# arangrhie/merfin

Measured on AMD Instinct MI355X. Metric: k-mers evaluated/sec (-hist, k=21), higher is better.
Workload: dtype u64 k-mers / u32 counts / f64 K*

## Files before the change

include/merfin_amd.h:

```cpp
#ifndef MERFIN_AMD_H
#define MERFIN_AMD_H

#include <stddef.h>
#include <stdint.h>

#ifdef __cplusplus
extern "C" {
#endif

#define MFX_OK            0
#define MFX_E_INVAL      -1
#define MFX_E_NOMEM      -2
#define MFX_E_HIP        -3
#define MFX_E_FULL       -4
#define MFX_E_OVERFLOW   -5
#define MFX_E_IO         -6
#define MFX_E_FORMAT     -7
#define MFX_E_NODEVICE   -8
#define MFX_E_NONCANON   -9

const char *mfx_last_error(void);
int         mfx_last_error_code(void);
const char *mfx_version(void);
int         mfx_device_count(void);
// ... 150 lines not shown

typedef struct mfx_reads mfx_reads;
typedef struct mfx_reads_stats {
  uint64_t reads, bases;
  uint64_t kmers;
  uint64_t counted;
  uint64_t dropped;
  uint64_t saturated;
  double   seconds_kernel, seconds_copy;
} mfx_reads_stats;
mfx_reads *mfx_reads_begin(mfx_index *ix, uint64_t batch_bases);
int        mfx_reads_set_filter(mfx_reads *r, uint64_t minV, uint64_t maxV);
int        mfx_reads_add(mfx_reads *r, const char *const *bases, const uint64_t *lens, uint64_t n);
int        mfx_reads_end(mfx_reads *r, mfx_reads_stats *out);

mfx_reads *mfx_reads_begin_all(mfx_index *ix, uint64_t batch_bases);
mfx_reads *mfx_reads_begin_range(mfx_index *ix, uint64_t batch_bases, uint64_t key_lo, uint64_t key_hi);

typedef struct mfx_reads_store mfx_reads_store;
mfx_reads_store *mfx_reads_store_create(int k, uint64_t batch_bases, uint64_t max_bytes);
int  mfx_reads_store_add(mfx_reads_store *s, const char *const *bases, const uint64_t *lens, uint64_t n);
int  mfx_reads_store_info(const mfx_reads_store *s, uint64_t *batches, uint64_t *bytes, uint64_t *reads, uint64_t *n_bases, int *complete);
int  mfx_reads_replay(mfx_reads *r, const mfx_reads_store *s, uint64_t first_batch, uint64_t n_batches);
void mfx_reads_store_free(mfx_reads_store *s);
int        mfx_index_growths(const mfx_index *ix, uint64_t *n, double *seconds, double *rehash_seconds, uint64_t *rehash_bytes);

mfx_seq *mfx_seq_upload(int device, const char *const *bases, const uint64_t *lens, uint32_t ncontigs);
mfx_seq *mfx_seq_from_device(int device, const void *const *d_bases, const uint64_t *lens, uint32_t ncontigs,
                             void *stream);
void     mfx_seq_free(mfx_seq *s);
uint32_t mfx_seq_num_contigs(const mfx_seq *s);
uint64_t mfx_seq_num_bases(const mfx_seq *s);
uint64_t mfx_seq_num_tiles(const mfx_seq *s);
int      mfx_seq_is_packed(const mfx_seq *s);

typedef struct {
  double          peak;
  uint32_t        n_prob;
  const uint32_t *probK;
  const double   *probP;
} mfx_kparams;

typedef struct mfx_eval mfx_eval;

mfx_eval *mfx_eval_create(const mfx_index *ix, const mfx_kparams *kp, uint32_t nbins);
void      mfx_eval_free(mfx_eval *ev);
uint32_t  mfx_eval_nbins(const mfx_eval *ev);
int       mfx_diag_gather_rate(int device, uint64_t table_bytes, double *lines_per_s);
int       mfx_eval_debug_enable(mfx_eval *ev, int on);
int       mfx_eval_debug_counters(mfx_eval *ev, uint64_t *out8);
int       mfx_eval_debug_worklist(mfx_eval *ev, int mode, uint32_t segcap);
int       mfx_eval_debug_worklist_read(mfx_eval *ev, int slot, uint32_t *segs, uint32_t *segcap, uint64_t *counts, uint64_t counts_cap,
                                       void *entries, uint64_t entries_cap, uint64_t *n_entries);

int mfx_debug_traverse_host(const void *clusters, uint64_t ncl, const void *variants, uint64_t nvar, const void *alleles, uint64_t nal,
                            const char *win_text, uint64_t win_bytes, const char *al_text, uint64_t al_bytes, uint64_t text_end,
                            uint64_t path_cap, uint64_t row_cap, uint32_t *np, uint32_t *status, char *text, uint64_t *p_off,
                            uint32_t *p_len, uint32_t *p_nv, uint64_t *p_voff, uint64_t *p_cfirst, int32_t *gt, uint32_t *vidx,
                            uint32_t *vlen);
int mfx_debug_score_paths(mfx_eval *ev, const char *text, uint64_t len, uint64_t npaths, uint64_t nvals, const uint64_t *off,
                          const uint32_t *plen, const uint32_t *nv, const uint64_t *voff, const uint64_t *cfirst, const int32_t *gt,
                          const uint32_t *vidx, const uint32_t *vlen, int need_dk, uint32_t *numM, double *totdk);
int mfx_debug_score_paths_trv(mfx_eval *ev, const char *text, uint64_t len, uint64_t npaths, uint64_t nvals, const uint64_t *off,
                              const uint32_t *plen, const uint32_t *nv, const uint64_t *voff, const uint64_t *cfirst, const int32_t *gt,
                              const uint32_t *vidx, const uint32_t *vlen, const void *clusters, uint64_t ncl, const void *variants,
                              uint64_t nvar, const void *alleles, uint64_t nal, const char *win_text, uint64_t win_bytes,
                              const char *al_text, uint64_t al_bytes, uint64_t text_end, uint64_t path_cap, uint64_t row_cap, int need_dk,
                              uint32_t *numM, double *totdk, uint32_t *np, uint32_t *status, char *text_out, uint64_t *p_off,
                              uint32_t *p_len, uint32_t *p_nv, uint64_t *p_voff, uint64_t *p_cfirst, int32_t *gt_out, uint32_t *vidx_out,
                              uint32_t *vlen_out);

void mfx_getK(const mfx_kparams *kp, uint32_t readV, uint32_t asmV,
              double *readK, double *asmK, double *prob);
double mfx_getKmetric(double readK, double asmK);
double mfx_histoQV(double kval, double ktot, int k);

typedef struct {
  uint64_t  kasm;
  uint64_t  kmissing;
  double    koverCpy;
  uint32_t  undrMax, overMax;
  uint64_t *undr, *over;
  uint32_t  ncontigs;
  uint64_t *contig_kasm;
  uint64_t *contig_kmissing;
} mfx_hist_result;

int  mfx_hist_run(mfx_eval *ev, const mfx_seq *seq, mfx_hist_result *out);
void mfx_hist_result_free(mfx_hist_result *r);

void    *mfx_host_alloc(size_t bytes);
void     mfx_host_free(void *p);
mfx_seq *mfx_seq_create(int device, const uint64_t *lens, uint32_t ncontigs);
int      mfx_hist_run_streamed(mfx_eval *ev, mfx_seq *seq, const char *const *bases, mfx_hist_result *out);
int      mfx_hist_run_streamed_multi(mfx_eval *const *evs, mfx_seq *const *seqs, uint32_t ndev, const char *const *bases, mfx_hist_result *out);
int      mfx_hist_run_streamed_range(mfx_eval *ev, mfx_seq *seq, const char *const *bases, uint64_t tile_begin, uint64_t tile_end,
                                     uint64_t *d_counts, double *d_kover);
int      mfx_hist_stream_share(uint64_t ntiles, uint32_t rank, uint32_t nranks, uint64_t *tile_begin, uint64_t *tile_end);
int      mfx_diag_stream_rates(int device, const char *src, uint64_t n, uint32_t threads, double *enc_gbs, double *link_gbs);
void     mfx_pack_bases(const uint8_t *src, uint64_t n, uint64_t *codes, uint32_t *valid);

mfx_index *mfx_index_replicate(const mfx_index *src, int device);
mfx_seq   *mfx_seq_replicate(const mfx_seq *src, int device);
int        mfx_index_replicate_many(const mfx_index *src, const int *devices, uint32_t n, mfx_index **out);
int        mfx_seq_replicate_many(const mfx_seq *src, const int *devices, uint32_t n, mfx_seq **out);
int        mfx_seq_pack(mfx_seq *seq);
// ... 179 lines not shown
```

merfin_amd/binding.py:

```python
import ctypes as C
import os

import numpy as np

_HERE = os.path.dirname(os.path.abspath(__file__))
TILE = 4096

MFX_ERRORS = {-1: "INVAL", -2: "NOMEM", -3: "HIP", -4: "FULL", -5: "OVERFLOW", -6: "IO", -7: "FORMAT", -8: "NODEVICE", -9: "NONCANON"}
E_NONCANON = -9


class MfxError(RuntimeError):
    def __init__(self, code, msg):
        super().__init__("merfin_amd error %s (%d): %s" % (MFX_ERRORS.get(code, "?"), code, msg))
        self.code = code


def lib_path():
    return os.environ.get("MFX_LIB") or os.path.join(_HERE, "libmerfin_amd.so")


class _KP(C.Structure):
    _fields_ = [("peak", C.c_double), ("n_prob", C.c_uint32),
                ("probK", C.POINTER(C.c_uint32)), ("probP", C.POINTER(C.c_double))]
# ... 3 lines not shown
    _fields_ = [("k", C.c_int), ("canonical", C.c_int), ("capacity", C.c_uint64),
                ("distinct", C.c_uint64), ("bytes", C.c_uint64), ("seq_only", C.c_int), ("compact", C.c_int),
                ("dropped", C.c_uint64)]


class _DbInfo(C.Structure):
    _fields_ = [("k", C.c_int), ("format", C.c_int), ("n_kmers", C.c_uint64), ("placed", C.c_int)]


class _VarOpts(C.Structure):
    _fields_ = [("mode", C.c_int), ("comb", C.c_uint32), ("nosplit", C.c_int), ("debug_path", C.c_char_p)]


INDEX_HEADER_BYTES = 128

VARIANT_MODES = {"filter": 4, "polish": 5, "better": 6, "strict": 7, "loose": 8}


class _ReadsStats(C.Structure):
    _fields_ = [("reads", C.c_uint64), ("bases", C.c_uint64), ("kmers", C.c_uint64), ("counted", C.c_uint64),
                ("dropped", C.c_uint64), ("saturated", C.c_uint64), ("seconds_kernel", C.c_double), ("seconds_copy", C.c_double)]


class _SpectrumPeak(C.Structure):
    _fields_ = [("valley", C.c_uint32), ("main_peak", C.c_uint32), ("haploid_peak", C.c_uint32), ("count_at_peak", C.c_uint64)]


class _HistResult(C.Structure):
    _fields_ = [("kasm", C.c_uint64), ("kmissing", C.c_uint64), ("koverCpy", C.c_double),
                ("undrMax", C.c_uint32), ("overMax", C.c_uint32),
                ("undr", C.POINTER(C.c_uint64)), ("over", C.POINTER(C.c_uint64)),
                ("ncontigs", C.c_uint32),
                ("contig_kasm", C.POINTER(C.c_uint64)), ("contig_kmissing", C.POINTER(C.c_uint64))]


_lib = None

SYMBOLS = [
    "mfx_last_error", "mfx_last_error_code", "mfx_version", "mfx_device_count", "mfx_device_warm", "mfx_device_memory",
    "mfx_index_create", "mfx_index_free", "mfx_index_estimate_gb", "mfx_index_add_read", "mfx_index_add_asm",
    "mfx_index_count_asm", "mfx_index_build_for_hist", "mfx_index_count_claimed", "mfx_hist_run_parts", "mfx_index_create_for_seq", "mfx_index_create_for_seq_lf", "mfx_index_create_lf", "mfx_db_stage_begin", "mfx_index_build_for_hist_staged", "mfx_index_load_db_staged", "mfx_db_stage_free", "mfx_db_stage_boost", "mfx_index_estimate_gb_for_seq", "mfx_index_claim_seq", "mfx_index_value", "mfx_index_get_info", "mfx_index_export",
    "mfx_db_probe", "mfx_index_load_db", "mfx_index_load_db_multi", "mfx_db_write_flat", "mfx_db_convert", "mfx_db_merge", "mfx_db_merge_plan", "mfx_db_join_completeness", "mfx_db_join_spectrum", "mfx_db_join_grain", "mfx_db_join_host", "mfx_db_convert_placed", "mfx_db_write_flat_placed", "mfx_db_place_keys", "mfx_index_save", "mfx_index_load",
    "mfx_index_set_fingerprint", "mfx_index_get_origin",
    "mfx_host_alloc", "mfx_host_free", "mfx_seq_create", "mfx_hist_run_streamed",
    "mfx_hist_run_streamed_multi", "mfx_hist_run_streamed_range", "mfx_hist_stream_share",
    "mfx_index_replicate", "mfx_seq_replicate", "mfx_hist_run_multi", "mfx_hist_run_sharded",
    "mfx_comm_unique_id", "mfx_comm_create", "mfx_comm_free", "mfx_comm_rank", "mfx_comm_size", "mfx_comm_barrier", "mfx_comm_exchange_counts", "mfx_comm_alltoallv",
    "mfx_index_replicate_many", "mfx_seq_replicate_many", "mfx_seq_pack",
    "mfx_hist_allreduce", "mfx_hist_allgather_overflow", "mfx_hist_result_add_overflow",
    "mfx_index_image_header", "mfx_index_create_from_header", "mfx_index_device_image", "mfx_index_commit",
    "mfx_seq_upload", "mfx_seq_from_device", "mfx_seq_free", "mfx_seq_num_contigs", "mfx_seq_num_bases",
    "mfx_seq_num_tiles", "mfx_seq_is_packed",
    "mfx_diag_gather_rate",
    "mfx_eval_create", "mfx_eval_free", "mfx_eval_nbins", "mfx_eval_debug_enable", "mfx_eval_debug_counters", "mfx_eval_debug_worklist", "mfx_eval_debug_worklist_read", "mfx_getK", "mfx_getKmetric", "mfx_histoQV",
    "mfx_hist_run", "mfx_hist_result_free", "mfx_hist_launch", "mfx_hist_launch_cyclic", "mfx_hist_result_from_counts",
    "mfx_hist_take_overflow", "mfx_hist_report", "mfx_diag_stream_rates",
    "mfx_pack_bases", "mfx_host_threads_share", "mfx_dump_values", "mfx_dump_contig", "mfx_dump_values_sharded", "mfx_dump_contig_sharded", "mfx_variants_run_sharded", "mfx_vcf_load", "mfx_vcf_free", "mfx_variants_run_vcf", "mfx_vcf_prepare", "mfx_vcf_path_bound", "mfx_index_claim_paths", "mfx_vcf_prepare_path_index", "mfx_completeness", "mfx_completeness_pieces", "mfx_variants_run",
    "mfx_index_set_shard", "mfx_router_create", "mfx_router_free", "mfx_route_tiles", "mfx_hist_keys_launch",
    "mfx_reads_begin", "mfx_reads_set_filter", "mfx_reads_add", "mfx_reads_end",
    "mfx_reads_begin_all", "mfx_index_growths", "mfx_index_write_db",
    "mfx_reads_begin_range", "mfx_index_key_bins", "mfx_db_writer_open", "mfx_db_writer_append_index", "mfx_db_writer_close", "mfx_db_writer_abort",
    "mfx_db_writer_open_streamed", "mfx_db_writer_append_sorted", "mfx_db_writer_info", "mfx_index_write_db_streamed",
    "mfx_reads_store_create", "mfx_reads_store_add", "mfx_reads_store_info", "mfx_reads_replay", "mfx_reads_store_free",
    "mfx_track_num_windows", "mfx_track_run", "mfx_track_write",
    "mfx_regions_run", "mfx_regions_count", "mfx_regions_tiles_revisited", "mfx_diag_regions_times", "mfx_regions_copy", "mfx_regions_free",
    "mfx_regions_write", "mfx_regions_from_planes_host",
    "mfx_db_merge_except", "mfx_phase_run", "mfx_phase_count", "mfx_phase_copy", "mfx_phase_contig_counts", "mfx_phase_free", "mfx_diag_phase_times", "mfx_phase_write",
    "mfx_phase_from_planes_host",
    "mfx_bin_begin", "mfx_bin_add", "mfx_bin_flush", "mfx_bin_ready", "mfx_bin_take", "mfx_bin_end", "mfx_bin_classify", "mfx_bin_plan_host",
    "mfx_spectrum_run", "mfx_spectrum_peak", "mfx_spectrum_write", "mfx_diag_spectrum_time",
    "mfx_db_trio", "mfx_db_trio_hist", "mfx_db_histogram", "mfx_db_histogram_write", "mfx_db_trio_host",
    "mfx_db_diploid", "mfx_db_diploid_host", "mfx_diploid_write_asm",
    "mfx_debug_traverse_host", "mfx_debug_score_paths", "mfx_debug_score_paths_trv",
]

TRV_CLUSTER_DTYPE = np.dtype([("win_off", "<u8"), ("win_len", "<u4"), ("nv", "<u4"), ("var0", "<u4"), ("path_cap", "<u4"),
                              ("text0", "<u8"), ("path0", "<u8"), ("row0", "<u8"), ("text_cap", "<u4"), ("pad", "<u4")])
TRV_VARIANT_DTYPE = np.dtype([("off", "<u4"), ("reflen", "<u4"), ("na", "<u4"), ("al0", "<u4")])
TRV_ALLELE_DTYPE = np.dtype([("off", "<u8"), ("len", "<u4"), ("pad", "<u4")])
assert (TRV_CLUSTER_DTYPE.itemsize, TRV_VARIANT_DTYPE.itemsize, TRV_ALLELE_DTYPE.itemsize) == (56, 16, 16)
TRV_OK, TRV_RANGE, TRV_ROOM = 0, 1, 2
TRV_MAX_NV, TRV_MAX_PATHS, TRV_MAX_LEN = 8, 64, 640

WORKLIST_DTYPE = np.dtype([("kmer", "<u8"), ("aux", "<u4"), ("w", "<u4")])
assert WORKLIST_DTYPE.itemsize == 16

TRACK_DTYPE = np.dtype([("n_kmers", "<u4"), ("n_missing", "<u4"), ("n_scored", "<u4"), ("n_pos", "<u4"), ("n_neg", "<u4"),
                        ("n_nonfinite", "<u4"), ("sum_readK", "<u8"), ("sum_asmK", "<u8"), ("sum_kstar_lo", "<u8"),
                        ("sum_kstar_hi", "<i8"), ("min_kstar", "<f8"), ("max_kstar", "<f8")])
assert TRACK_DTYPE.itemsize == 72

REGION_DTYPE = np.dtype([("contig", "<u4"), ("cls", "<u4"), ("start", "<u8"), ("end", "<u8"), ("n_kmers", "<u8"), ("sum_readK", "<u8"),
                         ("sum_asmK", "<u8"), ("ext_kstar", "<f8")])
assert REGION_DTYPE.itemsize == 56
REGION_CLASSES = ("missing", "collapsed", "expanded")


class _RegionsOpts(C.Structure):
    _fields_ = [("kstar", C.c_double), ("gap", C.c_uint64), ("min_kmers", C.c_uint64)]


PHASE_DTYPE = np.dtype([("contig", "<u4"), ("hap", "<u4"), ("start", "<u8"), ("end", "<u8"), ("n_hap", "<u8"), ("n_switch", "<u8"),
                        ("n_switch_runs", "<u8")])
assert PHASE_DTYPE.itemsize == 48


class _PhaseOpts(C.Structure):
# ... 81 lines not shown
    L.mfx_db_merge.argtypes = [C.POINTER(C.c_char_p), C.c_uint32, C.c_char_p, C.POINTER(DbMergeOpts), C.POINTER(DbMergeStats)]
    L.mfx_db_merge_except.argtypes = [C.POINTER(C.c_char_p), C.c_uint32, C.POINTER(C.c_char_p), C.c_uint32, C.c_char_p, C.POINTER(DbMergeOpts), C.POINTER(DbMergeStats),
                                      u64p]
    L.mfx_db_merge_plan.argtypes = [C.POINTER(u64p), u64p, C.c_uint32, C.c_int, C.c_uint64, u64p, C.c_uint64, u64p]
    L.mfx_db_join_completeness.argtypes = [C.c_char_p, C.c_char_p, C.POINTER(DbJoinOpts), f64p, f64p, C.POINTER(DbJoinStats)]
    L.mfx_db_join_spectrum.argtypes = [C.c_char_p, C.c_char_p, C.POINTER(DbJoinOpts), u64p, u64p, C.POINTER(DbJoinStats)]
    L.mfx_db_join_grain.argtypes = [C.POINTER(C.c_uint32), C.POINTER(C.c_uint32)]
    L.mfx_db_join_grain.restype = None
    L.mfx_db_join_host.argtypes = [u64p, C.POINTER(C.c_uint32), C.c_uint64, u64p, C.POINTER(C.c_uint32), C.c_uint64, u64p, C.POINTER(C.c_uint32), C.POINTER(C.c_uint32),
                                   C.c_uint64, u64p]
    L.mfx_db_trio.argtypes = [C.c_char_p, C.c_char_p, C.c_char_p, C.c_char_p, C.c_char_p, C.POINTER(DbTrioOpts), u64p, C.POINTER(DbTrioStats)]
    L.mfx_db_trio_hist.argtypes = [C.c_char_p, C.c_char_p, C.c_char_p, C.c_uint32, u64p, C.POINTER(DbTrioStats), C.c_int]
    L.mfx_db_histogram.argtypes = [C.c_char_p, C.c_uint32, u64p, u64p, C.c_int]
    L.mfx_db_histogram_write.argtypes = [u64p, C.c_uint32, C.c_char_p]
    L.mfx_db_trio_host.argtypes = [u64p, C.POINTER(C.c_uint32), C.c_uint64, u64p, C.POINTER(C.c_uint32), C.c_uint64, u64p, C.POINTER(C.c_uint32), C.c_uint64, C.c_int,
                                   C.c_uint32, C.c_uint32, C.c_uint32, C.c_uint32, u64p, C.POINTER(C.c_uint32), u64p, u64p, C.POINTER(C.c_uint32), u64p, u64p,
                                   C.POINTER(DbTrioStats)]
    L.mfx_db_diploid.argtypes = [C.c_char_p, C.c_char_p, C.c_char_p, C.POINTER(DbJoinOpts), u64p, u64p, u64p, C.POINTER(DbDiploidStats), f64p, f64p]
    L.mfx_db_diploid_host.argtypes = [u64p, C.POINTER(C.c_uint32), C.c_uint64, u64p, C.POINTER(C.c_uint32), C.c_uint64, u64p, C.POINTER(C.c_uint32), C.c_uint64, C.c_int,
                                      C.POINTER(DbJoinOpts), u64p, C.POINTER(C.c_uint32), C.POINTER(C.c_uint32), C.POINTER(C.c_uint32), C.c_uint64, u64p, u64p, u64p, u64p,
                                      C.POINTER(DbDiploidStats), f64p, f64p]
    L.mfx_diploid_write_asm.argtypes = [u64p, C.c_uint32, C.c_char_p]
    L.mfx_db_write_flat_placed.argtypes = [C.c_char_p, C.c_int, u64p, u32p, C.c_uint64]
    L.mfx_db_place_keys.argtypes = [C.c_int, vp, C.c_uint64, vp, C.c_int, C.c_int]
    L.mfx_index_load_db_multi.argtypes = [C.POINTER(vp), C.c_uint32, C.c_char_p, C.c_int, C.c_uint64, C.c_uint64]
    L.mfx_index_save.argtypes = [vp, C.c_char_p]
    L.mfx_index_load.restype = vp
    L.mfx_index_load.argtypes = [C.c_char_p, C.c_double, C.c_int]
    L.mfx_index_image_header.argtypes = [vp, vp]
    L.mfx_index_create_from_header.restype = vp
    L.mfx_index_create_from_header.argtypes = [vp, C.c_double, C.c_int]
    L.mfx_index_device_image.argtypes = [vp, C.POINTER(vp), u64p, C.POINTER(vp), u64p]
    L.mfx_index_commit.argtypes = [vp]
    L.mfx_seq_upload.restype = vp
    L.mfx_seq_upload.argtypes = [C.c_int, C.POINTER(C.c_char_p), u64p, C.c_uint32]
    L.mfx_seq_from_device.restype = vp
    L.mfx_seq_from_device.argtypes = [C.c_int, C.POINTER(vp), u64p, C.c_uint32, vp]
    L.mfx_seq_free.argtypes = [vp]
    L.mfx_seq_num_contigs.restype = C.c_uint32
    L.mfx_seq_num_contigs.argtypes = [vp]
    L.mfx_seq_num_bases.restype = C.c_uint64
    L.mfx_seq_num_bases.argtypes = [vp]
    L.mfx_seq_num_tiles.restype = C.c_uint64
    L.mfx_seq_num_tiles.argtypes = [vp]
    L.mfx_eval_create.restype = vp
    L.mfx_eval_create.argtypes = [vp, C.POINTER(_KP), C.c_uint32]
    L.mfx_eval_free.argtypes = [vp]
    L.mfx_eval_nbins.restype = C.c_uint32
    L.mfx_eval_nbins.argtypes = [vp]
    L.mfx_diag_gather_rate.argtypes = [C.c_int, C.c_uint64, C.POINTER(C.c_double)]
    L.mfx_eval_debug_enable.argtypes = [vp, C.c_int]
    L.mfx_eval_debug_counters.argtypes = [vp, u64p]
    L.mfx_eval_debug_worklist.argtypes = [vp, C.c_int, C.c_uint32]
    L.mfx_eval_debug_worklist_read.argtypes = [vp, C.c_int, u32p, u32p, u64p, C.c_uint64, vp, C.c_uint64, u64p]
    L.mfx_getK.argtypes = [C.POINTER(_KP), C.c_uint32, C.c_uint32, f64p, f64p, f64p]
    L.mfx_getKmetric.restype = C.c_double
    L.mfx_getKmetric.argtypes = [C.c_double, C.c_double]
    L.mfx_histoQV.restype = C.c_double
    L.mfx_histoQV.argtypes = [C.c_double, C.c_double, C.c_int]
    L.mfx_hist_run.argtypes = [vp, vp, C.POINTER(_HistResult)]
    L.mfx_hist_result_free.argtypes = [C.POINTER(_HistResult)]
    L.mfx_hist_launch.argtypes = [vp, vp, C.c_uint64, C.c_uint64, vp, vp, vp]
    L.mfx_hist_launch_cyclic.argtypes = [vp, vp, C.c_uint32, C.c_uint32, C.c_uint32, vp, vp, vp]
    L.mfx_hist_result_from_counts.argtypes = [C.c_uint32, u64p, C.c_double, C.c_uint32, C.POINTER(_HistResult)]
    L.mfx_hist_take_overflow.argtypes = [vp, u64p, C.c_uint64, u64p]
    L.mfx_diag_stream_rates.argtypes = [C.c_int, vp, C.c_uint64, C.c_uint32, C.POINTER(C.c_double), C.POINTER(C.c_double)]
    L.mfx_hist_report.argtypes = [C.POINTER(_HistResult), C.c_int, C.c_char_p, C.c_char_p]
    L.mfx_dump_values.argtypes = [vp, vp, C.c_uint32, C.c_uint64, C.c_uint64, u32p, u32p, u64p, u64p]
    L.mfx_dump_contig.argtypes = [vp, vp, C.c_uint32, C.c_char_p, C.c_char_p, C.c_int, u64p, u64p]
    L.mfx_dump_values_sharded.argtypes = [vp, vp, C.c_uint32, C.c_uint32, C.c_uint64, C.c_uint64, u32p, u32p, u64p, u64p]
    L.mfx_dump_contig_sharded.argtypes = [vp, vp, C.c_uint32, C.c_uint32, C.c_char_p, C.c_char_p, C.c_int, u64p, u64p]
    L.mfx_variants_run_sharded.argtypes = [vp, C.c_uint32, C.c_char_p, C.POINTER(C.c_char_p), C.POINTER(C.c_char_p), u64p, C.c_uint32,
                                           C.POINTER(_VarOpts), C.c_char_p, C.c_char_p, u64p]
    L.mfx_completeness.argtypes = [vp, f64p, f64p]
    L.mfx_completeness_pieces.argtypes = [vp, f64p, f64p]
    L.mfx_index_set_shard.argtypes = [vp, C.c_uint32, C.c_uint32]
    L.mfx_router_create.restype = vp
    L.mfx_router_create.argtypes = [vp, C.c_uint32, C.c_uint32]
    L.mfx_router_free.argtypes = [vp]
    L.mfx_route_tiles.argtypes = [vp, vp, C.c_uint64, C.c_uint64, C.c_uint32, vp, vp, vp, u64p, vp]
    L.mfx_hist_keys_launch.argtypes = [vp, vp, vp, C.c_uint64, C.c_uint32, vp, vp, vp]
    L.mfx_variants_run.argtypes = [vp, C.c_char_p, C.POINTER(C.c_char_p), C.POINTER(C.c_char_p), u64p, C.c_uint32,
                                   C.POINTER(_VarOpts), C.c_char_p, C.c_char_p, u64p]
    L.mfx_vcf_load.restype = vp
    L.mfx_vcf_load.argtypes = [C.c_char_p]
    L.mfx_vcf_free.restype = None
    L.mfx_vcf_free.argtypes = [vp]
    L.mfx_variants_run_vcf.argtypes = [vp, vp, C.POINTER(C.c_char_p), C.POINTER(C.c_char_p), u64p, C.c_uint32,
                                       C.POINTER(_VarOpts), C.c_char_p, C.c_char_p, u64p]
    L.mfx_vcf_prepare.argtypes = [vp, C.c_int, C.POINTER(C.c_char_p), C.POINTER(C.c_char_p), u64p, C.c_uint32, C.POINTER(_VarOpts)]
    L.mfx_vcf_path_bound.argtypes = [vp, u64p]
    L.mfx_index_claim_paths.argtypes = [vp, vp, u64p]
    L.mfx_vcf_prepare_path_index.argtypes = [vp, C.c_int, C.POINTER(C.c_char_p), C.POINTER(C.c_char_p), u64p, C.c_uint32, C.POINTER(_VarOpts), C.c_double, C.c_int, C.c_double,
                                             C.POINTER(vp)]
    L.mfx_index_set_fingerprint.argtypes = [vp, C.c_uint64]
    L.mfx_index_get_origin.argtypes = [vp, u64p, u64p, u64p]
    L.mfx_host_threads_share.restype = None
    L.mfx_host_threads_share.argtypes = [C.c_uint]
    L.mfx_pack_bases.restype = None
    L.mfx_pack_bases.argtypes = [vp, C.c_uint64, vp, vp]
    L.mfx_host_alloc.restype = vp
    L.mfx_host_alloc.argtypes = [C.c_size_t]
    L.mfx_host_free.restype = None
    L.mfx_host_free.argtypes = [vp]
    L.mfx_seq_create.restype = vp
    L.mfx_seq_create.argtypes = [C.c_int, u64p, C.c_uint32]
# ... 574 lines not shown
    def commit(self):
        _check(load_library().mfx_index_commit(self.h))

    def replicate(self, device):
        h = _need(load_library().mfx_index_replicate(self.h, device))
        ix = Index(0, 0, device=device, _handle=h)
        ix.k = self.k
        return ix

    def replicate_many(self, devices):
        devs = (C.c_int * len(devices))(*devices)
        out = (C.c_void_p * len(devices))()
        _check(load_library().mfx_index_replicate_many(self.h, devs, len(devices), out))
        res = []
        for d, h in zip(devices, out):
            ix = Index(0, 0, device=d, _handle=h)
            ix.k = self.k
            res.append(ix)
        return res

    def set_fingerprint(self, fp):
        _check(load_library().mfx_index_set_fingerprint(self.h, int(fp)))

    def origin(self):
        a, b, c = C.c_uint64(), C.c_uint64(), C.c_uint64()
        _check(load_library().mfx_index_get_origin(self.h, C.byref(a), C.byref(b), C.byref(c)))
        return a.value, b.value, c.value

    def add_read(self, kmers, values, minV=0, maxV=2**64 - 1):
        if isinstance(kmers, np.ndarray):
            kmers = np.ascontiguousarray(kmers, dtype=np.uint64)
            values = np.ascontiguousarray(values, dtype=np.uint32)
        pk, dev, _k1 = _ptr(kmers)
        pv, _, _k2 = _ptr(values)
        _check(load_library().mfx_index_add_read(self.h, pk, pv, len(kmers), minV, maxV, dev))

    def add_asm(self, kmers, values):
        if isinstance(kmers, np.ndarray):
            kmers = np.ascontiguousarray(kmers, dtype=np.uint64)
            values = np.ascontiguousarray(values, dtype=np.uint32)
        pk, dev, _k1 = _ptr(kmers)
        pv, _, _k2 = _ptr(values)
        _check(load_library().mfx_index_add_asm(self.h, pk, pv, len(kmers), dev))

    def set_shard(self, rank, nranks):
        _check(load_library().mfx_index_set_shard(self.h, rank, nranks))

    def load_db(self, path, side, minV=0, maxV=2**64 - 1):
        _check(load_library().mfx_index_load_db(self.h, path.encode(), side, minV, maxV))

    def count_asm(self, seqs, stream=None):
        _check(load_library().mfx_index_count_asm(self.h, seqs.h, C.c_void_p(stream or 0)))

    def count_reads(self, reads, batch_bases=0, minV=0, maxV=2**64 - 1, chunk=4096):
        return self._count_reads(load_library().mfx_reads_begin, reads, batch_bases, minV, maxV, chunk)

    def count_reads_all(self, reads, batch_bases=0, chunk=4096, minV=0, maxV=2**64 - 1):
        return self._count_reads(load_library().mfx_reads_begin_all, reads, batch_bases, minV, maxV, chunk)

    def count_reads_range(self, reads, key_lo, key_hi, batch_bases=0, chunk=4096):
        L = load_library()
        return self._count_reads(lambda h, bb: L.mfx_reads_begin_range(h, bb, int(key_lo), int(key_hi)), reads, batch_bases, 0, 2**64 - 1, chunk)

    def key_bins(self, side=0):
        bins = np.zeros(4096, dtype=np.uint64)
        n = C.c_uint32(0)
        _check(load_library().mfx_index_key_bins(self.h, int(side), bins.ctypes.data_as(C.POINTER(C.c_uint64)), C.byref(n)))
        return bins[:n.value].copy()

    def growths(self):
        n, b = C.c_uint64(0), C.c_uint64(0)
        s, rs = C.c_double(0), C.c_double(0)
        _check(load_library().mfx_index_growths(self.h, C.byref(n), C.byref(s), C.byref(rs), C.byref(b)))
        return {"growths": n.value, "seconds": s.value, "rehash_seconds": rs.value, "rehash_bytes": b.value}

    def write_db(self, path, side=0, streamed=False):
        n = C.c_uint64(0)
        L = load_library()
        _check((L.mfx_index_write_db_streamed if streamed else L.mfx_index_write_db)(self.h, int(side), str(path).encode(), C.byref(n)))
        return n.value

    def _count_reads(self, begin, reads, batch_bases, minV, maxV, chunk):
        L = load_library()
        recs = [x.encode() if isinstance(x, str) else bytes(x) for x in reads]
        r = _need(begin(self.h, int(batch_bases)))
        rc = L.mfx_reads_set_filter(r, int(minV), int(maxV))
        for o in range(0, len(recs), chunk):
            if rc:
                break
            part = recs[o:o + chunk]
            ptrs = (C.c_char_p * len(part))(*part)
            lens = (C.c_uint64 * len(part))(*[len(x) for x in part])
            try:
                rc = L.mfx_reads_add(r, ptrs, lens, len(part))
            except BaseException:
                L.mfx_reads_end(r, None)
                raise
        msg = L.mfx_last_error().decode() if rc else ""
        st = _ReadsStats()
        rc_end = L.mfx_reads_end(r, C.byref(st))
        if rc:
            raise MfxError(rc, msg)
        _check(rc_end)
        return {f: getattr(st, f) for f, _ in _ReadsStats._fields_}

    def value(self, kmers):
# ... 715 lines not shown
        arr = (C.c_char_p * n)(*contigs)
        lens = np.array([len(c) for c in contigs], dtype=np.uint64)
        o = _VarOpts(VARIANT_MODES[mode], comb, 1 if nosplit else 0, debug_path.encode() if debug_path else None)
        h = C.c_void_p(None)
        _check(load_library().mfx_vcf_prepare_path_index(self.h, int(k), nm, arr, lens.ctypes.data_as(C.POINTER(C.c_uint64)), n, C.byref(o), float(max_gb), int(device),
                                                         float(load_factor), C.byref(h)))
        if not h.value:
            return None
        ix = Index(0, 0, device=device, _handle=h.value)
        ix.k = int(k)
        return ix

    def path_bound(self):
        n = C.c_uint64(0)
        _check(load_library().mfx_vcf_path_bound(self.h, C.byref(n)))
        return n.value

    def claim_paths(self, index):
        n = C.c_uint64(0)
        _check(load_library().mfx_index_claim_paths(index.h, self.h, C.byref(n)))
        return n.value

    def close(self):
        if self.h:
            load_library().mfx_vcf_free(self.h)
            self.h = None

    def __del__(self):
        try:
            self.close()
        except Exception:
            pass


class Evaluator:

    def __init__(self, index, kparams, nbins=0):
        self.index = index
        self.kp = kparams
        self.h = _need(load_library().mfx_eval_create(index.h, C.byref(kparams.c), nbins))

    @property
    def nbins(self):
        return load_library().mfx_eval_nbins(self.h)

    def debug(self, on=True):
        _check(load_library().mfx_eval_debug_enable(self.h, 1 if on else 0))

    def debug_counters(self):
        out = np.zeros(8, dtype=np.uint64)
        _check(load_library().mfx_eval_debug_counters(self.h, out.ctypes.data_as(C.POINTER(C.c_uint64))))
        return {"first_pass": int(out[0]), "second_pass": int(out[1]), "side_table": int(out[2]), "line_scans": int(out[3]),
                "side_not_in_two_slots": int(out[4]), "ended_per_lane": int(out[5]),
                "second_bucket": int(out[6])}

    def debug_worklist(self, mode=1, segcap=0):
        _check(load_library().mfx_eval_debug_worklist(self.h, mode, segcap))

    def debug_worklist_read(self, slot=0):
        L = load_library()
        segs, segcap, n = C.c_uint32(0), C.c_uint32(0), C.c_uint64(0)
        _check(L.mfx_eval_debug_worklist_read(self.h, slot, C.byref(segs), C.byref(segcap), None, 0, None, 0, C.byref(n)))
        counts = np.zeros(segs.value, dtype=np.uint64)
        ent = np.zeros(n.value, dtype=WORKLIST_DTYPE)
        _check(L.mfx_eval_debug_worklist_read(self.h, slot, C.byref(segs), C.byref(segcap), counts.ctypes.data_as(C.POINTER(C.c_uint64)), len(counts),
                                              C.c_void_p(ent.ctypes.data), len(ent), C.byref(n)))
        assert n.value == len(ent) and segs.value == len(counts)
        return segs.value, segcap.value, counts, ent

    def hist(self, seqs):
        r = HistResult()
        _check(load_library().mfx_hist_run(self.h, seqs.h, C.byref(r.c)))
        return r

    def hist_streamed(self, seqs, host_contigs):
        ptrs, keep = _host_ptrs(host_contigs)
        r = HistResult()
        _check(load_library().mfx_hist_run_streamed(self.h, seqs.h, ptrs, C.byref(r.c)))
        return r

    def hist_streamed_range(self, seqs, host_contigs, tile_begin, tile_end, d_counts, d_kover):
        ptrs, keep = _host_ptrs(host_contigs)
        pc = d_counts.data_ptr() if hasattr(d_counts, "data_ptr") else int(d_counts)
        pk = d_kover.data_ptr() if hasattr(d_kover, "data_ptr") else int(d_kover)
        _check(load_library().mfx_hist_run_streamed_range(self.h, seqs.h, ptrs, tile_begin, tile_end, C.c_void_p(pc), C.c_void_p(pk)))

    def hist_launch(self, seqs, tile_begin, tile_end, d_counts, d_kover, stream=None):
        pc = d_counts.data_ptr() if hasattr(d_counts, "data_ptr") else int(d_counts)
        pk = d_kover.data_ptr() if hasattr(d_kover, "data_ptr") else int(d_kover)
        _check(load_library().mfx_hist_launch(self.h, seqs.h, tile_begin, tile_end, C.c_void_p(pc), C.c_void_p(pk),
                                              C.c_void_p(stream or 0)))

    def hist_launch_cyclic(self, seqs, rank, nranks, d_counts, d_kover, block_tiles=256, stream=None):
        p = lambda x: C.c_void_p(x.data_ptr() if hasattr(x, "data_ptr") else int(x))
        _check(load_library().mfx_hist_launch_cyclic(self.h, seqs.h, rank, nranks, block_tiles, p(d_counts), p(d_kover),
                                                     C.c_void_p(stream or 0)))

    def result_from_counts(self, h_counts, kover, ncontigs):
        return result_from_counts(self.nbins, h_counts, kover, ncontigs)

    def take_overflow(self, cap=1 << 20):
        rec = np.zeros(2 * cap, dtype=np.uint64)
        n = C.c_uint64(0)
        _check(load_library().mfx_hist_take_overflow(self.h, rec.ctypes.data_as(C.POINTER(C.c_uint64)), cap, C.byref(n)))
        return rec[:2 * n.value].reshape(-1, 2)

    def hist_keys_launch(self, d_keys, d_contigs, n, ncontigs, d_counts, d_kover, stream=None):
# ... 150 lines not shown
```

merfin_amd/csrc/mfx_api.cpp:

```cpp
#include "mfx_host.h"
#include "mfx_histsum.h"
#include "mfx_place.h"
#include "mfx_kernels.h"
#include "mfx_pipe.h"
#include "mfx_pool.h"
#include "mfx_stream_plan.h"

#include <math.h>
#include <stdarg.h>
#include <stddef.h>
#include <stdio.h>
#include <stdlib.h>
#include <string.h>
#include <unistd.h>

#include <algorithm>
#include <atomic>
#include <chrono>
#include <memory>
#include <mutex>
#include <functional>
#include <condition_variable>
#include <string>
#include <thread>
#include <unordered_map>
#include <vector>

static thread_local char g_err[1024] = "";
static thread_local int  g_err_code = 0;

void mfx_set_error(const char *fmt, ...) {
  va_list ap;
  va_start(ap, fmt);
  vsnprintf(g_err, sizeof(g_err), fmt, ap);
  va_end(ap);
}

int mfx_fail(int code, const char *fmt, ...) {
  va_list ap;
  va_start(ap, fmt);
  vsnprintf(g_err, sizeof(g_err), fmt, ap);
  va_end(ap);
  g_err_code = code;
  return code;
}

extern "C" const char *mfx_last_error(void) { return g_err; }
extern "C" int mfx_last_error_code(void) { return g_err_code; }
extern "C" const char *mfx_version(void) { return "merfin_amd 0.2 (gfx950)"; }

extern "C" int mfx_diag_gather_rate(int device, uint64_t table_bytes, double *lines_per_s) {
  if (!lines_per_s || table_bytes < (1ull << 20)) return mfx_fail(MFX_E_INVAL, "mfx_diag_gather_rate: bad argument");
  if (device < 0 || device >= mfx_device_count()) return mfx_fail(MFX_E_NODEVICE, "HIP device %d not available", device);
  int prev = -1;
  (void)hipGetDevice(&prev);
  MFX_HIP(hipSetDevice(device));
// ... 259 lines not shown
    if (budget > 0) budget = std::max(1.0, budget - (double)ix->side_nlines * MFX_ALIGN);
    ix->nlines = lines_auto(capacity_kmers, budget, slots_line, seq_only);
    if (ix->quot) ix->nlines = std::max(ix->nlines, quot_min_lines(k));
  }
  if (ix->nlines >= (1ull << 32)) {
    mfx_fail(MFX_E_NOMEM, "Not enough memory to load databases.  %lu k-mers need %.0f GB on one GPU; shard the index (mfx_index_set_shard).",
             (unsigned long)capacity_kmers, (double)ix->nlines * MFX_ALIGN / 1e9);
    delete ix;
    return nullptr;
  }
  {
    const char *hm = getenv("MFX_HOME_MODE");
    bool mz = hm ? (strcmp(hm, "plain") != 0) : true;
    const char *ws = getenv("MFX_MZ_W");
    const int w_default = compact ? MFX_MZ_W_COMPACT : MFX_MZ_W_DEFAULT;
    int w = ws ? atoi(ws) : w_default;
    if (w < 1 || w > 5) w = w_default;
    ix->mz_w = (mz && !ix->wide()) ? std::min(w, k) : 0;
    {
      const char *mm = getenv("MFX_MZ_MOD");
      const bool modw = ix->mz_w == 4 || (ix->mz_w == 5 && !ix->quot);
      ix->mz_t = (compact && modw && k >= 13 && !(mm && atoi(mm) == 0)) ? (ix->mz_w == 4 ? ((k + 1) & 3) + 4 : 4 + ((k - 8) % 5)) : 0;
    }
  }
  hipError_t e = hipMalloc((void **)&ix->d_slots, ix->total_lines() * MFX_ALIGN);
  if (e != hipSuccess && ix->nlines > std::max(lines_for(capacity_kmers, slots_line), quot_min_lines(ix->quot ? k : 0))) {
    (void)hipGetLastError();
    ix->nlines = std::max(lines_for(capacity_kmers, slots_line), quot_min_lines(ix->quot ? k : 0));
    e = hipMalloc((void **)&ix->d_slots, ix->total_lines() * MFX_ALIGN);
  }
  if (e != hipSuccess) {
    mfx_fail(MFX_E_NOMEM, "hipMalloc of %.3f GB for the k-mer table failed: %s", need, hipGetErrorString(e));
    delete ix;
    return nullptr;
  }
  if (hipMalloc((void **)&ix->d_meta, MFX_META_WORDS * sizeof(uint64_t)) != hipSuccess ||
      mfx_memset_now(ix->d_meta, 0, MFX_META_WORDS * sizeof(uint64_t)) != hipSuccess ||
      (ix->wide() ? hipMemsetAsync(ix->d_slots, 0, ix->nlines * MFX_ALIGN, nullptr)
       : ix->compact ? hipMemsetAsync(ix->d_slots, 0xff, ix->nlines * MFX_ALIGN, nullptr)
                     : mfx_k_table_init(ix->d_slots, ix->nlines * MFX_SLOTS_LINE, nullptr)) != hipSuccess ||
      (ix->compact && mfx_k_table_init(ix->d_slots + ix->nlines * MFX_SLOTS_LINE, ix->side_nlines * MFX_SLOTS_LINE, nullptr) != hipSuccess) ||
      hipDeviceSynchronize() != hipSuccess) {
    mfx_fail(MFX_E_HIP, "k-mer table initialisation failed: %s", hipGetErrorString(hipGetLastError()));
    mfx_index_free(ix);
    return nullptr;
  }
  return ix;
}

extern "C" void mfx_index_free(mfx_index *ix) {
  if (!ix) return;
  DevGuard g(ix->device);
  mfx_index_ingest_release(ix);
  if (ix->d_slots) (void)hipFree(ix->d_slots);
  if (ix->d_meta) (void)hipFree(ix->d_meta);
  delete ix;
}

static mfx_ingest *ingest_get(mfx_index *ix, uint64_t n);

static int index_check(mfx_index *ix) {
  ix->version++;
  uint64_t meta[5];
  MFX_HIP(hipMemcpy(meta, ix->d_meta, sizeof(meta), hipMemcpyDeviceToHost));
  if (meta[4] != 0)
    return mfx_fail(MFX_E_FORMAT, "the database holds %lu records wider than 2k = %d bits: damaged or not a %d-mer database (none was inserted)",
                    (unsigned long)meta[4], 2 * ix->k, ix->k);
  if (meta[2] != 0)
    return mfx_fail(MFX_E_FULL, "k-mer table full: %lu inserts hit the probe limit (capacity %lu k-mers, %lu stored)",
                    (unsigned long)meta[2], (unsigned long)ix->capacity_kmers, (unsigned long)meta[0]);
  if ((double)meta[0] > 0.92 * (double)(ix->nlines * ix->slots_per_line()))
    return mfx_fail(MFX_E_FULL, "k-mer table over-full: %lu k-mers in %lu slots; create the index with a larger capacity",
                    (unsigned long)meta[0], (unsigned long)(ix->nlines * ix->slots_per_line()));
  if (ix->seq_only && meta[1] != 0)
    return mfx_fail(MFX_E_NONCANON, "the database holds %lu non-canonical k-mers: a sequence-only index keeps one slot per canonical k-mer of the "
                    "sequence and cannot answer value(fmer) + value(rmer) for it; build a full index (mfx_index_create)", (unsigned long)meta[1]);
  return MFX_OK;
}

int mfx_index_check(mfx_index *ix) { return index_check(ix); }

int mfx_reads_claim_error(const mfx_index *ix, const char *who) {
  return mfx_fail(MFX_E_INVAL, "%s: reads were counted into this table of %d-mers (mfx_reads_begin); a table of k > %d claims every k-mer it is "
                  "given, and one claimed now would lack the reads' counts -- give the assembly side before the reads", who, ix->k, MFX_MAX_K_NARROW);
}

constexpr uint64_t MFX_INGEST_CHUNK = 1ull << 24;
constexpr int MFX_INGEST_MAX_LANES = 4, MFX_INGEST_MAX_RING = 64, MFX_INGEST_STREAMS = 4;
struct mfx_ingest {
  struct Lane {
    uint64_t *hk = nullptr;
    uint32_t *hv = nullptr;
    hipEvent_t copied = nullptr;
    bool busy = false;
  } L[MFX_INGEST_MAX_LANES];
  struct Dev {
    uint64_t *dk = nullptr;
    uint32_t *dv = nullptr;
    hipEvent_t done = nullptr;
    bool busy = false;
  } D[MFX_INGEST_MAX_RING];
  hipStream_t cs = nullptr;
  hipStream_t is[MFX_INGEST_STREAMS] = {nullptr, nullptr, nullptr, nullptr};
  hipEvent_t after = nullptr;
  int nl = 2;
  int nd = 2;
// ... 294 lines not shown
    if (!par_pread(fd, (uint8_t *)hk, bytes, off(b0), pool.get())) { mfx_fail(MFX_E_IO, "reading '%s' failed", path); return -1; }
    memcpy(hv, dir + 2 * b0, (nb + 1) * 16);
    const uint64_t base = off(b0), m = std::min<uint64_t>(n - b0 * MFX_DELTA_BLOCK, nb * MFX_DELTA_BLOCK);
    d.kbytes = bytes;
    d.vbytes = (nb + 1) * 16;
    d.launch = [nb, m, base, side, placed](mfx_index *ix, uint64_t *dk, uint32_t *dv, hipStream_t st) {
      return placed ? mfx_k_table_add_placed(ix->view(), dk, reinterpret_cast<const uint64_t *>(dv), (uint32_t)nb, m, base, side, ix->d_meta, st)
                    : mfx_k_table_add_delta(ix->view(), dk, reinterpret_cast<const uint64_t *>(dv), (uint32_t)nb, m, base, side, ix->d_meta, st);
    };
    b0 = b1;
    return 1;
  });
}

static int index_add(mfx_index *ix, const uint64_t *kmers, const uint32_t *values, uint64_t n, int side, int on_device) {
  if (!ix || (n && (!kmers || !values))) return mfx_fail(MFX_E_INVAL, "mfx_index_add: null argument");
  if (ix->reads_counted && ix->wide()) return mfx_reads_claim_error(ix, "mfx_index_add");
  DevGuard g(ix->device);
  const size_t kw = ix->key_words();
  auto table_add = [&](const uint64_t *dk, const uint32_t *dv, uint64_t m, hipStream_t s) {
    return ix->wide() ? mfx_kw_table_add(ix->view(), dk, dv, m, side, ix->d_meta, s) : mfx_k_table_add(ix->view(), dk, dv, m, side, ix->d_meta, s);
  };
  if (on_device) {
    ix->frozen = true;
    MFX_HIP(table_add(kmers, values, n, nullptr));
    MFX_HIP(hipDeviceSynchronize());
    return index_check(ix);
  }
  return index_ingest(ix, n, side, [&](uint64_t o, uint64_t m, uint64_t *hk, uint32_t *hv) {
    par_memcpy((uint8_t *)hk, (const char *)(kmers + o * kw), m * 8 * kw);
    par_memcpy((uint8_t *)hv, (const char *)(values + o), m * 4);
    return true;
  });
}

extern "C" int mfx_index_add_read(mfx_index *ix, const uint64_t *kmers, const uint32_t *values, uint64_t n,
                                  uint64_t minV, uint64_t maxV, int on_device) {
  if (!ix) return mfx_fail(MFX_E_INVAL, "mfx_index_add_read: null index");
  if (ix->reads_counted)
    return mfx_fail(MFX_E_INVAL, "mfx_index_add_read: the read side of this index was counted from reads (mfx_reads_begin); an index takes its "
                    "read counts from one source");
  if (ix->filter_set && (ix->minV != minV || ix->maxV != maxV))
    return mfx_fail(MFX_E_INVAL, "mfx_index_add_read: -min/-max must be the same for every batch of one index");
  ix->minV = minV;
  ix->maxV = maxV;
  ix->filter_set = true;
  return index_add(ix, kmers, values, n, 0, on_device);
}

extern "C" int mfx_index_add_asm(mfx_index *ix, const uint64_t *kmers, const uint32_t *values, uint64_t n, int on_device) {
  return index_add(ix, kmers, values, n, 1, on_device);
}

static int index_count(mfx_index *ix, const mfx_seq *seq, int count, void *stream, const char *who, bool defer = false, bool no_wait = false) {
  if (!ix || !seq) return mfx_fail(MFX_E_INVAL, "%s: null argument", who);
  if (ix->device != seq->device) return mfx_fail(MFX_E_INVAL, "index and sequence live on different devices");
  if (ix->reads_counted && ix->wide()) return mfx_reads_claim_error(ix, who);
  if (ix->seq_only && ix->frozen && count != 2)
    return mfx_fail(MFX_E_INVAL, "%s: this sequence-only index already took counts; its k-mers must all be claimed before the first add / load "
                    "(a k-mer claimed now would have missed them)", who);
  if (count == 2 && (!ix->seq_only || ix->wide())) return mfx_fail(MFX_E_INVAL, "%s: counting claimed k-mers needs a sequence-only index (mfx_index_create_for_seq)", who);
  if (seq->partial) return mfx_seq_partial_error(seq, who);
  const bool from_planes = !ix->wide() && (seq->planes_ok || seq->bases_stale) && !(getenv("MFX_COUNT_ASCII") && atoi(getenv("MFX_COUNT_ASCII")));
  if (!from_planes) if (int erc = mfx_seq_ensure_ascii(seq)) return erc;
  DevGuard g(ix->device);
  mfx_count_args a;
  a.t = ix->view();
  a.bases = seq->d_bases;
  if (from_planes) { a.codes = seq->d_codes; a.valid = seq->d_valid; }
  a.contig_off = seq->d_contig_off;
  a.contig_len = seq->d_contig_len;
  a.tile_start = seq->d_tile_start;
  a.ncontigs = seq->ncontigs;
  a.ntiles = seq->ntiles;
  a.meta = ix->d_meta;
  a.count = count;
  if (ix->seq_only && count != 2) {
    uint32_t d = 0;
    if (int drc = mfx_seq_digest32(seq, &d)) return drc;
    if (ix->seq_digest != 0 && ix->seq_digest != d)
      return mfx_fail(MFX_E_INVAL, "%s: this sequence-only index already claimed the k-mers of another sequence (content digest %08x, this one %08x); "
                      "one such index answers for ONE sequence object -- put the contigs into one mfx_seq", who, ix->seq_digest, d);
    ix->seq_digest = d;
  }
  if (count == 2) ix->frozen = true;
  MFX_HIP(ix->wide() ? mfx_kw_count(a, (hipStream_t)stream) : mfx_k_count(a, (hipStream_t)stream));
  if (no_wait) return MFX_OK;
  if (defer) {
    hipEvent_t ev = nullptr;
    hipError_t e = hipEventCreateWithFlags(&ev, hipEventDisableTiming);
    if (e == hipSuccess) e = hipEventRecord(ev, (hipStream_t)stream);
    mfx_ingest *g = e == hipSuccess ? ingest_get(ix, 1ull << 22) : nullptr;
    if (g) {
      if (g->after) { (void)hipEventSynchronize(g->after); (void)hipEventDestroy(g->after); }
      g->after = ev;
      return MFX_OK;
    }
    if (ev) (void)hipEventDestroy(ev);
    (void)hipGetLastError();
  } else if (ix->seq_only && seq->total_bases >= (256ull << 20)) (void)ingest_get(ix, 1ull << 22);
  MFX_HIP(hipStreamSynchronize((hipStream_t)stream));
  return index_check(ix);
}

static void ingest_settle_after(mfx_index *ix) {
  if (!ix || !ix->ingest || !ix->ingest->after) return;
  DevGuard g(ix->device);
  (void)hipEventSynchronize(ix->ingest->after);
  (void)hipEventDestroy(ix->ingest->after);
  ix->ingest->after = nullptr;
}

extern "C" int mfx_index_count_asm(mfx_index *ix, const mfx_seq *seq, void *stream) {
  return index_count(ix, seq, 1, stream, "mfx_index_count_asm");
}

extern "C" int mfx_index_count_claimed(mfx_index *ix, const mfx_seq *seq, void *stream) {
  return index_count(ix, seq, 2, stream, "mfx_index_count_claimed");
}

extern "C" int mfx_index_build_for_hist(mfx_index *ix, const mfx_seq *seq, const char *read_db_path, uint64_t minV, uint64_t maxV) {
  if (!ix || !seq || !read_db_path) return mfx_fail(MFX_E_INVAL, "mfx_index_build_for_hist: null argument");
  const char *ov = getenv("MFX_BUILD_OVERLAP");
  const bool defer = !(ov && atoi(ov) == 0);
  int rc = index_count(ix, seq, 1, nullptr, "mfx_index_build_for_hist", defer);
  if (rc == MFX_OK) rc = mfx_index_load_db(ix, read_db_path, 0, minV, maxV);
  ingest_settle_after(ix);
  return rc;
}

struct mfx_db_stage {
  int device = 0, fd = -1;
  std::string path;
  mfx_flat_delta_info info;
  std::vector<uint64_t> dir;
  uint64_t off0 = 0, payload_bytes = 0;
  uint8_t *d_payload = nullptr;
  uint64_t *d_dir = nullptr;
// ... 367 lines not shown
      std::fill(tc.begin() + (size_t)s->tile_start[c], tc.begin() + (size_t)s->tile_start[c + 1], c);
    MFX_HIP(hipMalloc((void **)&s->d_tile_contig, (tc.size() ? tc.size() : 1) * sizeof(uint32_t)));
    if (!tc.empty()) MFX_HIP(hipMemcpy(s->d_tile_contig, tc.data(), tc.size() * sizeof(uint32_t), hipMemcpyHostToDevice));
  }
  return MFX_OK;
}


int mfx_seq_partial_error(const mfx_seq *s, const char *who) {
  return mfx_fail(MFX_E_INVAL, "%s: the sequence object holds only the tiles [%lu, %lu) of its %lu (the part one device evaluated in a streamed run over "
                  "several); upload the sequence whole", who, (unsigned long)s->part_lo, (unsigned long)s->part_hi, (unsigned long)s->ntiles);
}

int mfx_seq_ensure_ascii(const mfx_seq *cs) {
  if (cs && cs->partial) return mfx_seq_partial_error(cs, "unpacking the sequence");
  std::lock_guard<std::mutex> lazy(cs->lazy_mu);
  if (!cs->bases_stale && cs->d_bases) return MFX_OK;
  mfx_seq *s = const_cast<mfx_seq *>(cs);
  DevGuard g(s->device);
  if (int rc = seq_need_bases(s)) return rc;
  if (!s->bases_stale) return MFX_OK;
  MFX_HIP(mfx_k_unpack(s->d_codes, s->d_valid, s->d_bases, s->buf_bytes / 32, nullptr));
  MFX_HIP(hipDeviceSynchronize());
  s->bases_stale = false;
  return MFX_OK;
}

void seq_digest_finish(const mfx_seq *s, uint64_t h) {
  for (uint32_t c = 0; c < s->ncontigs; ++c) h = (h ^ s->len[c]) * 0x100000001B3ULL + c;
  const uint32_t f = (uint32_t)(h ^ (h >> 32));
  s->digest = f ? f : 1u;
}

int mfx_seq_digest32(const mfx_seq *s, uint32_t *out) {
  if (s->partial) return mfx_seq_partial_error(s, "the sequence's content digest");
  std::lock_guard<std::mutex> lazy(s->lazy_mu);
  if (s->digest == 0) {
    DevGuard g(s->device);
    uint64_t *d = nullptr, h = 0;
    MFX_HIP(hipMalloc((void **)&d, sizeof(uint64_t)));
    hipError_t e = mfx_memset_now(d, 0, sizeof(uint64_t));
    const bool planes = s->planes_ok || s->bases_stale;
    if (!planes && !s->d_bases) { (void)hipFree(d); if (int rc = seq_need_bases(const_cast<mfx_seq *>(s))) return rc; MFX_HIP(hipMalloc((void **)&d, sizeof(uint64_t))); e = mfx_memset_now(d, 0, sizeof(uint64_t)); }
    if (e == hipSuccess) e = mfx_k_seq_digest(s->d_bases, planes ? s->d_codes : nullptr, planes ? s->d_valid : nullptr, s->buf_bytes / 32, d, nullptr);
    if (e == hipSuccess) e = hipMemcpy(&h, d, sizeof(h), hipMemcpyDeviceToHost);
    (void)hipFree(d);
    if (e != hipSuccess) return mfx_fail(MFX_E_HIP, "sequence digest failed: %s", hipGetErrorString(e));
    seq_digest_finish(s, h);
  }
  *out = s->digest;
  return MFX_OK;
}

thread_local bool t_mfx_path_lookup = false;
int mfx_check_seq_of_index(const mfx_index *ix, const mfx_seq *s, const char *who) {
  if (!ix->seq_only || ix->seq_digest == 0) return MFX_OK;
  if (ix->paths_token) {
    if (t_mfx_path_lookup) return MFX_OK;
    return mfx_fail(MFX_E_INVAL, "%s: this index holds the k-mers of a variant call set's PATHS (mfx_index_claim_paths) and answers the variant modes of that "
                    "call set only; build the index from the sequence (mfx_index_create_for_seq) or use a full index", who);
  }
  uint32_t d = 0;
  if (int rc = mfx_seq_digest32(s, &d)) return rc;
  if (d != ix->seq_digest)
    return mfx_fail(MFX_E_INVAL, "%s: this sequence-only index holds the k-mers of ANOTHER sequence (content digest %08x, this one %08x): "
                    "k-mers it never claimed would read as absent; build the index from this sequence (mfx_index_create_for_seq + "
                    "mfx_index_count_asm / mfx_index_claim_seq) or use a full index", who, ix->seq_digest, d);
  return MFX_OK;
}

static void seq_pack_resident(mfx_seq *s) {
  const char *e = getenv("MFX_SEQ_PACK");
  if ((e && atoi(e) == 0) || !s->d_bases) return;
  const bool timing = getenv("MFX_UPLOAD_TIMING") != nullptr;
  const auto t0 = std::chrono::steady_clock::now();
  const uint64_t pw = seq_plane_words(s);
  const bool ok = mfx_seq_planes_once(
      s, pw,
      [](void **p, size_t bytes) { const bool got = hipMalloc(p, bytes) == hipSuccess; if (!got) { *p = nullptr; (void)hipGetLastError(); } return got; },
      [](void *p) { (void)hipFree(p); },
      [pw](mfx_seq *q) {
        const bool done = mfx_memset_now(q->d_valid, 0, pw * sizeof(uint32_t)) == hipSuccess &&
                          mfx_memset_now(q->d_codes, 0, pw * sizeof(uint64_t)) == hipSuccess &&
                          mfx_k_pack(q->d_bases, q->d_codes, q->d_valid, q->buf_bytes / 32, nullptr) == hipSuccess && hipDeviceSynchronize() == hipSuccess;
        if (!done) (void)hipGetLastError();
        return done;
      });
  if (timing)
    fprintf(stderr, "-- resident sequence: packed planes %s, %.3f s (%.1f MB)\n", ok ? "made" : "NOT made (evaluated from its bytes)",
            std::chrono::duration<double>(std::chrono::steady_clock::now() - t0).count(), pw * 12 / 1e6);
}

extern "C" mfx_seq *mfx_seq_upload(int device, const char *const *bases, const uint64_t *lens, uint32_t ncontigs) {
  if ((ncontigs && (!bases || !lens)) || device < 0 || device >= mfx_device_count()) {
    mfx_fail(device < 0 || device >= mfx_device_count() ? MFX_E_NODEVICE : MFX_E_INVAL,
             "mfx_seq_upload: bad argument (device %d of %d)", device, mfx_device_count());
    return nullptr;
  }
  DevGuard g(device);
  const double t_up0 = std::chrono::duration<double>(std::chrono::steady_clock::now().time_since_epoch()).count();
  mfx_seq *s = seq_layout(device, lens, ncontigs);
  const double t_up1 = std::chrono::duration<double>(std::chrono::steady_clock::now().time_since_epoch()).count();
  bool packed_transport = false;
  {
    const char *asc = getenv("MFX_UPLOAD_ASCII");
    const char *pm = getenv("MFX_UPLOAD_PACKED_MIN");
// ... 297 lines not shown
  if (ntl == 0) return MFX_OK;
  DevGuard g(ev->device);
  int canon = 0;
  int rc = eval_canonical(ev, &canon);
  if (rc) return rc;
  if (!chunk_of_total) {
    if (seq->partial) return mfx_seq_partial_error(seq, "-hist");
    rc = mfx_check_seq_of_index(ev->ix, seq, "-hist");
    if (rc) return rc;
  }
  const char *force = getenv("MFX_FORCE_TWO_STRAND");
  if (force && atoi(force)) canon = 0;
  if (!chunk_of_total) {
    rc = ensure_tile_partials(ev, ntl);
    if (rc) return rc;
  }
  if (seq->bases_stale && ev->ix->wide()) {
    rc = mfx_seq_ensure_ascii(seq);
    if (rc) return rc;
  }
  if (!(seq->planes_ok || seq->bases_stale) && !seq->d_bases) {
    rc = mfx_seq_ensure_ascii(seq);
    if (rc) return rc;
  }
  mfx_hist_args a;
  a.t = ev->ix->view();
  a.canonical = canon;
  a.bases = seq->d_bases;
  if (seq->planes_ok || seq->bases_stale) { a.codes = seq->d_codes; a.valid = seq->d_valid; }
  a.contig_off = seq->d_contig_off;
  a.contig_len = seq->d_contig_len;
  a.tile_start = seq->d_tile_start;
  a.ncontigs = seq->ncontigs;
  a.tile_begin = tile_begin;
  a.tile_end = tile_end;
  a.tile_contig = seq->d_tile_contig;
  a.tile_ctr = ev->d_tile_ctr + ctr_slot;
  a.tile_partials = ev->d_tile_partials + (chunk_of_total ? (tile_begin - partials_tile0) * (MFX_BLOCK / 64) : 0);
  a.n_logical = ntl;
  a.part_rank = part_rank;
  a.part_n = part_n;
  a.part_shift = part_shift;
  a.ks.peak = ev->peak;
  a.ks.n_prob = ev->n_prob;
  a.ks.probK = ev->d_probK;
  a.ks.probP = ev->d_probP;
  a.ks.underq = ev->d_underq;
  a.ks.nbins = ev->nbins;
  a.ks.ncontigs = seq->ncontigs;
  a.ks.counts = d_counts;
  a.ks.partials = ev->d_partials;
  a.ks.ovf = ev->d_ovf;
  a.dbg = ev->d_dbg;
  const char *wl_env = getenv("MFX_HIST_WORKLIST");
  const bool wl_off = (wl_env && atoi(wl_env) == 0) || ev->dbg_wl_mode == 0;
  ev->wl_used_segs[ctr_slot] = ev->wl_used_segcap[ctr_slot] = 0;
  if (a.t.compact && canon && ntl < (1ull << 27) && !wl_off) {
    rc = ensure_worklist(ev, ctr_slot, chunk_of_total ? std::max<uint64_t>(ntl, std::min<uint64_t>(chunk_of_total, (128ull << 20) / MFX_TILE)) : ntl);
    if (rc) return rc;
    const uint64_t segs = std::min<uint64_t>((uint64_t)ev->grid, ntl);
    if (ev->d_wl[ctr_slot] && segs <= MFX_WL_HEADER - 2) {
      a.wl = ev->d_wl[ctr_slot];
      a.wl_segs = (uint32_t)segs;
      a.wl_segcap = (uint32_t)(ev->wl_cap[ctr_slot] / segs);
      if (ev->dbg_wl_mode == 2) a.wl_segcap = std::min(a.wl_segcap, ev->dbg_wl_segcap);
      ev->wl_used_segs[ctr_slot] = a.wl_segs;
      ev->wl_used_segcap[ctr_slot] = a.wl_segcap;
    }
  }
  MFX_HIP(ev->ix->wide() ? mfx_kw_hist(a, (int)std::min<uint64_t>((uint64_t)ev->grid, ntl), (hipStream_t)stream)
                          : mfx_k_hist(a, (int)std::min<uint64_t>((uint64_t)ev->grid, ntl), (hipStream_t)stream));
  if (a.wl) MFX_HIP(mfx_k_hist_rest(a, (int)(a.wl_segs * 4u), (hipStream_t)stream));
  if (chunk_of_total) MFX_HIP(hipMemsetAsync(ev->d_tile_ctr + ctr_slot, 0, sizeof(uint64_t), (hipStream_t)stream));
  else MFX_HIP(mfx_k_sum_tile_partials(ev->d_tile_partials, ntl, d_kover, ev->d_tile_ctr, (hipStream_t)stream, ev->ix->wide() ? 0 : 1));
  return MFX_OK;
}

extern "C" int mfx_hist_launch(mfx_eval *ev, const mfx_seq *seq, uint64_t tile_begin, uint64_t tile_end,
                               uint64_t *d_counts, double *d_kover, void *stream) {
  if (!ev || !seq || !d_counts || !d_kover) return mfx_fail(MFX_E_INVAL, "mfx_hist_launch: null argument");
  if (ev->device != seq->device) return mfx_fail(MFX_E_INVAL, "evaluator and sequence live on different devices");
  if (tile_begin > tile_end || tile_end > seq->ntiles) return mfx_fail(MFX_E_INVAL, "tile range [%lu,%lu) outside [0,%lu)",
                                                                      (unsigned long)tile_begin, (unsigned long)tile_end, (unsigned long)seq->ntiles);
  return hist_launch(ev, seq, tile_begin, tile_end, 0, 1, 0, d_counts, d_kover, stream);
}

extern "C" int mfx_hist_launch_cyclic(mfx_eval *ev, const mfx_seq *seq, uint32_t rank, uint32_t nranks, uint32_t block_tiles,
                                      uint64_t *d_counts, double *d_kover, void *stream) {
  if (!ev || !seq || !d_counts || !d_kover) return mfx_fail(MFX_E_INVAL, "mfx_hist_launch_cyclic: null argument");
  if (ev->device != seq->device) return mfx_fail(MFX_E_INVAL, "evaluator and sequence live on different devices");
  if (nranks == 0 || rank >= nranks || block_tiles == 0 || (block_tiles & (block_tiles - 1)))
    return mfx_fail(MFX_E_INVAL, "mfx_hist_launch_cyclic: rank %u of %u, block of %u tiles (a power of two)", rank, nranks, block_tiles);
  uint32_t shift = 0;
  while ((1u << shift) < block_tiles) ++shift;
  if (nranks == 1) return hist_launch(ev, seq, 0, seq->ntiles, 0, 1, 0, d_counts, d_kover, stream);
  return hist_launch(ev, seq, 0, seq->ntiles, rank, nranks, shift, d_counts, d_kover, stream);
}

hipError_t ovf_reset_hip(mfx_eval *ev, hipStream_t st) {
  const hipError_t e = hipMemsetAsync(ev->d_ovf, 0, (2 + (size_t)MFX_OVF_SLOTS) * sizeof(uint64_t), st);
  return e != hipSuccess ? e : hipMemsetAsync(ev->d_ovf + 2 + MFX_OVF_SLOTS, 0xff, (size_t)MFX_OVF_SLOTS * sizeof(uint64_t), st);
}
int mfx_ovf_reset_async(mfx_eval *ev, hipStream_t st) {
  MFX_HIP(ovf_reset_hip(ev, st));
  return MFX_OK;
}
// ... 1051 lines not shown
```

merfin_amd/csrc/mfx_debug.cpp:

```cpp
#include "mfx_internal.h"
#include "mfx_kernels.h"

#include <stddef.h>
#include <string.h>

static_assert(sizeof(mfx_trv_variant) == 16 && offsetof(mfx_trv_variant, off) == 0 && offsetof(mfx_trv_variant, reflen) == 4 &&
              offsetof(mfx_trv_variant, na) == 8 && offsetof(mfx_trv_variant, al0) == 12, "mfx_trv_variant: layout of the C ABI");
static_assert(sizeof(mfx_trv_allele) == 16 && offsetof(mfx_trv_allele, off) == 0 && offsetof(mfx_trv_allele, len) == 8 &&
              offsetof(mfx_trv_allele, pad) == 12, "mfx_trv_allele: layout of the C ABI");
static_assert(sizeof(mfx_trv_cluster) == 56 && offsetof(mfx_trv_cluster, win_off) == 0 && offsetof(mfx_trv_cluster, win_len) == 8 &&
              offsetof(mfx_trv_cluster, nv) == 12 && offsetof(mfx_trv_cluster, var0) == 16 && offsetof(mfx_trv_cluster, path_cap) == 20 &&
              offsetof(mfx_trv_cluster, text0) == 24 && offsetof(mfx_trv_cluster, path0) == 32 && offsetof(mfx_trv_cluster, row0) == 40 &&
              offsetof(mfx_trv_cluster, text_cap) == 48 && offsetof(mfx_trv_cluster, pad) == 52, "mfx_trv_cluster: layout of the C ABI");

namespace {

int check_tables(const char *who, const mfx_trv_cluster *cl, uint64_t ncl, const mfx_trv_variant *var, uint64_t nvar, const mfx_trv_allele *al, uint64_t nal,
                 uint64_t win_bytes, uint64_t al_bytes, uint64_t text_begin, uint64_t text_end, uint64_t path_cap, uint64_t row_cap, bool every_slot) {
  std::vector<uint8_t> owned(every_slot ? path_cap : 0, 0);
  for (uint64_t c = 0; c < ncl; ++c) {
    const mfx_trv_cluster &C = cl[c];
    if (C.win_off > win_bytes || C.win_len > win_bytes - C.win_off) return mfx_fail(MFX_E_INVAL, "%s: cluster %lu: window outside the window text", who, (unsigned long)c);
    if (C.var0 > nvar || C.nv > nvar - C.var0) return mfx_fail(MFX_E_INVAL, "%s: cluster %lu: variants outside the table", who, (unsigned long)c);
    if (C.text0 < text_begin || C.text0 > text_end || C.text_cap > text_end - C.text0) return mfx_fail(MFX_E_INVAL, "%s: cluster %lu: text room outside [%lu, %lu)", who, (unsigned long)c, (unsigned long)text_begin, (unsigned long)text_end);
// ... 100 lines not shown
  rb.p_off = p_off; rb.p_voff = p_voff; rb.p_cfirst = p_cfirst; rb.p_nv = p_nv;
  rb.vidx = vidx_out; rb.vlen = vlen_out;
  return mfx_score_paths_trv(ev, text, len, &pt, &tb, need_dk, numM, totdk, &rb);
}

extern "C" int mfx_eval_debug_worklist(mfx_eval *ev, int mode, uint32_t segcap) {
  if (!ev) return mfx_fail(MFX_E_INVAL, "mfx_eval_debug_worklist: null argument");
  if (mode < 0 || mode > 2) return mfx_fail(MFX_E_INVAL, "mfx_eval_debug_worklist: mode %d (0 no list, 1 default, 2 segments of at most segcap entries)", mode);
  if (mode == 2 && segcap == 0) return mfx_fail(MFX_E_INVAL, "mfx_eval_debug_worklist: mode 2 with segments of 0 entries (mode 0 turns the list off)");
  ev->dbg_wl_mode = mode;
  ev->dbg_wl_segcap = mode == 2 ? segcap : 0u;
  return MFX_OK;
}

extern "C" int mfx_eval_debug_worklist_read(mfx_eval *ev, int slot, uint32_t *segs, uint32_t *segcap, uint64_t *counts, uint64_t counts_cap, void *entries,
                                            uint64_t entries_cap, uint64_t *n_entries) {
  if (!ev || !segs || !segcap || !n_entries) return mfx_fail(MFX_E_INVAL, "mfx_eval_debug_worklist_read: null argument");
  if (slot < 0 || slot > 1) return mfx_fail(MFX_E_INVAL, "mfx_eval_debug_worklist_read: slot %d (0 or 1)", slot);
  *segs = ev->wl_used_segs[slot];
  *segcap = ev->wl_used_segcap[slot];
  *n_entries = 0;
  if (!*segs) return MFX_OK;
  const uint64_t S = *segs, SC = *segcap;
  if (!ev->d_wl[slot] || S > MFX_WL_HEADER - 2 || S * SC > ev->wl_cap[slot])
    return mfx_fail(MFX_E_INVAL, "mfx_eval_debug_worklist_read: %lu segments of %lu entries do not lie in the list of %lu entries", (unsigned long)S,
                    (unsigned long)SC, (unsigned long)ev->wl_cap[slot]);
  int prev = 0;
  MFX_HIP(hipGetDevice(&prev));
  MFX_HIP(hipSetDevice(ev->device));
  struct Back { int d; ~Back() { (void)hipSetDevice(d); } } back{prev};
  MFX_HIP(hipDeviceSynchronize());
  std::vector<uint64_t> n(S);
  MFX_HIP(hipMemcpy(n.data(), ev->d_wl[slot] + 2, S * sizeof(uint64_t), hipMemcpyDeviceToHost));
  uint64_t total = 0;
  for (uint64_t g = 0; g < S; ++g) {
    if (n[g] > SC) return mfx_fail(MFX_E_INVAL, "mfx_eval_debug_worklist_read: segment %lu counts %lu entries, beyond its %lu", (unsigned long)g, (unsigned long)n[g], (unsigned long)SC);
    total += n[g];
  }
  *n_entries = total;
  if (counts) {
    if (counts_cap < S) return mfx_fail(MFX_E_INVAL, "mfx_eval_debug_worklist_read: %lu segments, the caller's counts hold %lu", (unsigned long)S, (unsigned long)counts_cap);
    memcpy(counts, n.data(), S * sizeof(uint64_t));
  }
  if (entries) {
    if (entries_cap < total) return mfx_fail(MFX_E_INVAL, "mfx_eval_debug_worklist_read: %lu entries, the caller's buffer holds %lu", (unsigned long)total, (unsigned long)entries_cap);
    uint8_t *dst = static_cast<uint8_t *>(entries);
    for (uint64_t g = 0; g < S; ++g) {
      if (n[g]) MFX_HIP(hipMemcpy(dst, ev->d_wl[slot] + MFX_WL_HEADER + 2 * g * SC, n[g] * 16, hipMemcpyDeviceToHost));
      dst += n[g] * 16;
    }
  }
  return MFX_OK;
}
```

merfin_amd/csrc/mfx_internal.h:

```cpp
#pragma once
#include "mfx_traverse.h"

#include <hip/hip_runtime.h>
#include <stdint.h>
#include <mutex>
#include <string>
#include <vector>

#include "../../include/merfin_amd.h"
#include "mfx_kstar.h"
#include "mfx_delta.h"

void mfx_set_error(const char *fmt, ...);
int  mfx_fail(int code, const char *fmt, ...);
#define MFX_HIP(call)                                                                         \
  do {                                                                                        \
    hipError_t e_ = (call);                                                                   \
    if (e_ != hipSuccess)                                                                     \
      return mfx_fail(MFX_E_HIP, "%s failed: %s (%s:%d)", #call, hipGetErrorString(e_), __FILE__, __LINE__); \
  } while (0)
#define MFX_HIP_NULL(call)                                                                    \
  do {                                                                                        \
    hipError_t e_ = (call);                                                                   \
    if (e_ != hipSuccess) {                                                                   \
// ... 62 lines not shown
};
constexpr uint32_t MFX_WSLOTS_LINE = 4;
constexpr int      MFX_MAX_K_NARROW = 31, MFX_MAX_K = 64;

constexpr uint32_t MFX_CSLOTS_LINE = 16;
constexpr uint32_t MFX_CSAT = 2047u;
constexpr int      MFX_MAX_K_COMPACT = 31;
constexpr int      MFX_MAX_K_DIRECT = 21;
constexpr int      MFX_MZ_W_COMPACT = 4;

struct mfx_table_view {
  mfx_slot *slots;
  uint64_t  nlines;
  uint32_t  minV, maxV;
  int       k;
  int       mz_w;
  int       mz_t;
  uint32_t  shard_rank, shard_n;
  int       wide;
  int       seq_only;
  int       compact;
  int       quot;
  int       qshift;
  mfx_slot *side;
  uint64_t  side_nlines;
};

struct mfx_ingest;
struct WorkerPool;

struct mfx_index {
  int       device = 0;
  mfx_ingest *ingest = nullptr;
  int       k = 0;
  uint64_t  capacity_kmers = 0;
  uint64_t  nlines = 0;
  mfx_slot *d_slots = nullptr;
  uint64_t *d_meta = nullptr;
  uint64_t  minV = 0, maxV = ~0ull;
  bool      filter_set = false;
  int       mz_w = 0;
  int       mz_t = 0;
  uint32_t  shard_rank = 0, shard_n = 1;
  uint64_t  version = 0;
  uint64_t  fingerprint = 0;
  bool      seq_only = false;
  bool      compact = false;
  bool      quot = false;
  bool      frozen = false;
  bool      reads_counted = false;
  uint64_t  side_nlines = 0;
  uint64_t  paths_token = 0;
  uint32_t  seq_digest = 0;
  double    max_gb = 0;
  uint64_t  grow_count = 0, rehash_bytes = 0;
  double    grow_seconds = 0, rehash_seconds = 0;
  uint64_t  total_lines() const { return nlines + side_nlines; }
  bool      wide() const { return k > MFX_MAX_K_NARROW; }
  uint32_t  slots_per_line() const { return wide() ? MFX_WSLOTS_LINE : compact ? MFX_CSLOTS_LINE : MFX_SLOTS_LINE; }
  uint32_t  key_words() const { return wide() ? 2u : 1u; }
  mfx_table_view view() const;
};

struct mfx_seq {
  int       device = 0;
  uint32_t  ncontigs = 0;
  uint64_t  total_bases = 0;
  uint64_t  ntiles = 0;
  uint64_t  buf_bytes = 0;
  uint8_t  *d_bases = nullptr;
  uint64_t *d_codes = nullptr;
  uint32_t *d_valid = nullptr;
  bool      bases_stale = false;
  bool      planes_ok = false;
  uint64_t *d_contig_off = nullptr;
  uint64_t *d_contig_len = nullptr;
  uint64_t *d_tile_start = nullptr;
  uint32_t *d_tile_contig = nullptr;
  std::vector<uint64_t> off, len, tile_start;
  bool      partial = false;
  uint64_t  part_lo = 0, part_hi = 0;
  mutable std::mutex lazy_mu;
  mutable uint32_t digest = 0;
};

template <class Alloc, class Release, class Fill>
inline bool mfx_seq_planes_once(mfx_seq *s, uint64_t plane_words, Alloc alloc, Release release, Fill fill) {
  if (s->planes_ok || s->bases_stale) return true;
  void *c = s->d_codes, *v = s->d_valid;
  bool ok = (c || alloc(&c, plane_words * sizeof(uint64_t))) && (v || alloc(&v, plane_words * sizeof(uint32_t)));
  s->d_codes = static_cast<uint64_t *>(c);
  s->d_valid = static_cast<uint32_t *>(v);
  ok = ok && fill(s);
  if (!ok) {
    if (c) release(c);
    if (v) release(v);
    s->d_codes = nullptr;
    s->d_valid = nullptr;
  }
  s->planes_ok = ok;
  return ok;
}

int mfx_seq_digest32(const mfx_seq *s, uint32_t *out);
int mfx_check_seq_of_index(const mfx_index *ix, const mfx_seq *s, const char *who);
extern thread_local bool t_mfx_path_lookup;

struct mfx_path_table {
  uint64_t        npaths = 0, nvals = 0;
  const uint64_t *off = nullptr;
  const uint32_t *len = nullptr;
  const uint32_t *nv = nullptr;
  const uint64_t *voff = nullptr;
  const uint64_t *cfirst = nullptr;
  const int32_t  *gt = nullptr;
  const uint32_t *vidx = nullptr, *vlen = nullptr;
};
int mfx_score_paths(mfx_eval *ev, const char *text, uint64_t len, const mfx_path_table *pt, int need_dk, uint32_t *numM, double *totdk);

struct mfx_trv_batch {
  uint64_t ncl = 0, nvar = 0, nal = 0, win_bytes = 0, al_bytes = 0;
  const mfx_trv_cluster *cl = nullptr;
  const mfx_trv_variant *var = nullptr;
  const mfx_trv_allele *al = nullptr;
  const char *win_text = nullptr, *al_text = nullptr;
  uint64_t text_end = 0;
  uint64_t path_cap = 0, row_cap = 0;
  uint32_t *np = nullptr, *status = nullptr;
  uint32_t *p_len = nullptr;
  int32_t *gt = nullptr;
};
struct mfx_trv_readback {
  char *text = nullptr;
  uint64_t *p_off = nullptr, *p_voff = nullptr, *p_cfirst = nullptr;
  uint32_t *p_nv = nullptr, *vidx = nullptr, *vlen = nullptr;
};
int mfx_score_paths_trv(mfx_eval *ev, const char *text, uint64_t len, const mfx_path_table *pt, const mfx_trv_batch *tb, int need_dk, uint32_t *numM, double *totdk,
                        const mfx_trv_readback *rb = nullptr);

int  mfx_claim_paths_batch(mfx_index *ix, uint8_t **scratch, uint64_t *scratch_bytes, const char *text, uint64_t len, const mfx_trv_batch *tb, uint64_t *bad);
int  mfx_claim_paths_finish(mfx_index *ix, uint64_t token);
void mfx_claim_paths_release(int device, uint8_t *scratch);

int mfx_seq_partial_error(const mfx_seq *s, const char *who);
int mfx_seq_ensure_ascii(const mfx_seq *s);

struct mfx_eval {
  const mfx_index *ix = nullptr;
  int       device = 0;
  double    peak = 0;
  uint32_t  n_prob = 0;
  std::vector<uint32_t> probK;
  std::vector<double>   probP;
  uint32_t *d_probK = nullptr;
  double   *d_probP = nullptr;
  uint64_t *d_underq = nullptr;
  uint32_t  nbins = 65536;
// ... 37 lines not shown
```

merfin_amd/csrc/mfx_kernels.h:

```cpp
#pragma once
#include "mfx_internal.h"

struct mfx_kstar_args {
  double          peak;
  uint32_t        n_prob;
  const uint32_t *probK;
  const double   *probP;
  uint32_t        nbins;
  uint32_t        ncontigs;
  uint64_t       *counts;
  double         *partials;
  uint64_t       *ovf;
  const uint64_t *underq = nullptr;
};

constexpr uint32_t MFX_WL_HEADER = 4096 + 2;
struct mfx_hist_args {
  mfx_table_view  t;
  int             canonical;
  const uint8_t  *bases;
  const uint64_t *codes = nullptr;
  const uint32_t *valid = nullptr;
  const uint64_t *contig_off, *contig_len, *tile_start;
  uint32_t        ncontigs;
  uint64_t        tile_begin, tile_end;
  const uint32_t *tile_contig;
  uint64_t       *tile_ctr;
  double         *tile_partials;
  uint64_t        n_logical;
  uint32_t        part_rank, part_n, part_shift;
  uint64_t       *dbg = nullptr;
  uint64_t       *wl = nullptr;
  uint32_t        wl_segs = 0, wl_segcap = 0;
  mfx_kstar_args  ks;
};

struct mfx_route_args {
  mfx_table_view  t;
  const uint8_t  *bases;
  const uint64_t *contig_off, *contig_len, *tile_start;
  uint32_t        ncontigs;
  uint64_t        tile_begin, tile_end;
  uint32_t        nranks;
  uint64_t       *keys;
  uint8_t        *owner;
  uint64_t       *dest_counts;
  uint64_t       *counts;
  uint32_t        nbins;
  const uint32_t *tile_contig;
  uint32_t       *tile_cnt;
};

constexpr uint32_t MFX_KEYS_MAX_SEGS = 16;
struct mfx_hist_keys_args {
  mfx_table_view  t;
  const uint64_t *keys = nullptr;
  const uint32_t *contig = nullptr;
  uint64_t        n = 0;
  uint32_t        nseg = 0;
  const uint64_t *seg_keys[MFX_KEYS_MAX_SEGS] = {};
  const uint32_t *seg_contig[MFX_KEYS_MAX_SEGS] = {};
  uint64_t        seg_n[MFX_KEYS_MAX_SEGS] = {};
  uint64_t       *kfix = nullptr;
  mfx_kstar_args  ks;
};

struct mfx_dump_args {
  mfx_table_view  t;
  int             canonical;
  const uint8_t  *src;
  uint64_t        npos;
  uint64_t        skip;
  uint64_t        clen_left;
  uint32_t       *readV, *asmV;
  double          peak;
  uint32_t        n_prob;
  const uint32_t *probK;
  const double   *probP;
  uint64_t       *stats;
  int             recount = 0;
};

struct mfx_track_args {
  mfx_table_view  t;
  int             canonical;
  const uint8_t  *bases;
// ... 19 lines not shown
  const uint64_t *codes = nullptr;
  const uint32_t *valid = nullptr;
  const uint64_t *contig_off, *contig_len, *tile_start;
  const uint32_t *tile_contig;
  uint64_t        ntiles;
  double          peak;
  uint32_t        n_prob;
  const uint32_t *probK;
  const double   *probP;
  double          kstar;
  uint64_t       *planes;
  uint64_t       *stats = nullptr;
  const uint64_t *tile_flag = nullptr;
  uint64_t       *regs = nullptr;
  uint64_t       *recount = nullptr;
  uint64_t        reg_begin0 = 0, reg_begin1 = 0, reg_begin2 = 0, reg_begin3 = 0;
};

struct mfx_phase_args {
  mfx_table_view  t;
  int             canonical;
  const uint8_t  *bases;
  const uint64_t *codes = nullptr;
  const uint32_t *valid = nullptr;
  const uint64_t *contig_off, *contig_len, *tile_start;
  const uint32_t *tile_contig;
  uint64_t        ntiles;
  uint64_t       *planes;
  uint64_t       *counts;
};

struct mfx_bin_args {
  mfx_table_view  t;
  int             canonical;
  const uint64_t *codes;
  const uint32_t *valid;
  uint64_t        npos;
  const uint64_t *piece_start;
  const uint64_t *tile_first;
  uint64_t        npieces;
  uint64_t       *out;
};

struct mfx_count_args {
  mfx_table_view  t;
  const uint8_t  *bases;
  const uint64_t *codes = nullptr;
  const uint32_t *valid = nullptr;
  const uint64_t *contig_off, *contig_len, *tile_start;
  uint32_t        ncontigs;
  uint64_t        ntiles;
  uint64_t       *meta;
  int             count = 1;
};

struct mfx_reads_args {
  mfx_table_view  t;
  const uint64_t *codes;
  const uint32_t *valid;
  uint64_t        npos;
  uint64_t       *meta;
  uint64_t       *stats;
  uint64_t        key_lo = 0, key_hi = 0;
};

struct mfx_var_score_args {
  const uint8_t  *text;
  const uint32_t *readV, *asmV;
  uint64_t        npaths;
  const uint64_t *off;
  const uint32_t *len, *nv;
  const uint64_t *voff;
  const uint64_t *cfirst;
  const int32_t  *gt;
  const uint32_t *vidx, *vlen;
  uint32_t        k;
  int             need_dk;
  double          peak;
  uint32_t        n_prob;
  const uint32_t *probK;
  const double   *probP;
  uint32_t       *numM;
  double         *totdk;
};
hipError_t mfx_k_var_score(const mfx_var_score_args &a, hipStream_t st);
hipError_t mfx_k_var_traverse(const mfx_trv_cluster *cl, uint64_t ncl, const mfx_trv_variant *vars, const mfx_trv_allele *alleles, const char *win_text,
                              const char *allele_text, const mfx_trv_out &o, uint32_t *np, uint32_t *status, hipStream_t st);
hipError_t mfx_k_table_init(mfx_slot *slots, uint64_t nslots, hipStream_t st);
hipError_t mfx_k_table_add(mfx_table_view t, const uint64_t *kmers, const uint32_t *values, uint64_t n, int side,
                           uint64_t *meta, hipStream_t st);
hipError_t mfx_k_table_add_delta(mfx_table_view t, const uint64_t *payload, const uint64_t *dir, uint32_t nblocks, uint64_t n,
                                 uint64_t payload_base, int side, uint64_t *meta, hipStream_t st);
hipError_t mfx_k_table_add_placed(mfx_table_view t, const uint64_t *payload, const uint64_t *dir, uint32_t nblocks, uint64_t n,
                                  uint64_t payload_base, int side, uint64_t *meta, hipStream_t st);
int        mfx_k_table_takes_placed(const mfx_table_view &t);
hipError_t mfx_k_place_keys(int k, const uint64_t *kmers, uint64_t n, uint64_t *out, hipStream_t st);
hipError_t mfx_k_table_value(mfx_table_view t, const uint64_t *kmers, uint64_t n, uint32_t *readV, uint32_t *asmV,
                             hipStream_t st);
hipError_t mfx_k_table_export(mfx_table_view t, uint64_t *kmers, uint32_t *readV, uint32_t *asmV,
                              unsigned long long *count, hipStream_t st);
hipError_t mfx_k_hist(const mfx_hist_args &a, int grid, hipStream_t st);
hipError_t mfx_k_route(const mfx_route_args &a, hipStream_t st);
hipError_t mfx_k_route_split(const mfx_route_args &a, uint64_t *keys_out, uint32_t *contig_out, hipStream_t st);
hipError_t mfx_k_route_gather(const mfx_route_args &a, const uint32_t *idx, uint64_t nvalid, uint64_t *keys_out,
                              uint32_t *contig_out, hipStream_t st);
hipError_t mfx_k_iota(uint32_t *v, uint64_t n, hipStream_t st);
// ... 108 lines not shown
```

merfin_amd/csrc/mfx_kernels.hip:

```cpp
#include "mfx_internal.h"
#include "mfx_kernels.h"
#include "mfx_device.h"
#include "mfx_place.h"
#include "mfx_track.h"
#define MFX_REGIONS_DEVICE
#include "mfx_regions.h"
#define MFX_PHASE_DEVICE
#include "mfx_phase.h"
#include "mfx_spectrum.h"

#include <stdlib.h>
#include <algorithm>

__device__ __forceinline__ uint64_t mfx_revcomp(uint64_t fwd, int k) {
  uint64_t x = __brevll(fwd) >> (64 - 2 * k);
  x = ((x & 0x5555555555555555ULL) << 1) | ((x >> 1) & 0x5555555555555555ULL);
  uint64_t mask = (~0ULL) >> (64 - 2 * k);
  return (x ^ 0xAAAAAAAAAAAAAAAAULL) & mask;
}


constexpr uint32_t MFX_MZ_REGION = 4;
constexpr uint32_t MFX_MAX_LINES = 512;

struct mfx_probe {
  uint32_t lineA, lineB;
  uint32_t b0;
  uint64_t fkey;
};

__device__ __forceinline__ uint64_t mfx_minimizer(uint64_t key, uint64_t rc, int k, int w) {
  const int m = k - w + 1;
  const uint64_t mmask = (~0ULL) >> (64 - 2 * m);
  uint64_t best = 0;
  uint32_t best_o = 0;
#pragma unroll
  for (int j = 0; j < 5; ++j) {
    if (j < w) {
      uint64_t a = (key >> (2 * j)) & mmask;
      uint64_t b = (rc >> (2 * (w - 1 - j))) & mmask;
      uint64_t c = a < b ? a : b;
      uint32_t o = ((uint32_t)c ^ (uint32_t)(c >> 32)) * 0x9E3779B1u;
      const bool take = (j == 0) || (o < best_o);
      best = take ? c : best;
      best_o = take ? o : best_o;
    }
  }
  return best;
}

__device__ __forceinline__ uint32_t mfx_tmer_order(uint32_t canonical_tmer) { return ((canonical_tmer * 0x9E3779B1u) >> 7) & 511u; }

__device__ __forceinline__ void mfx_mod_window(uint64_t key, uint64_t rc, int k, int w, int t, uint32_t &x, uint64_t &wa, uint64_t &wb) {
  const uint32_t tmask = (1u << (2 * t)) - 1u;
  uint32_t best = 0xffffffffu;
// ... 304 lines not shown
    const uint4 *ln = reinterpret_cast<const uint4 *>(t.slots + mfx_probe_line(t, pr, d) * MFX_SLOTS_LINE);
    bool any_empty = false;
#pragma unroll 1
    for (uint32_t q = 0; q < MFX_SLOTS_LINE; ++q) {
      const uint4 s = ln[q];
      const uint64_t sk = (uint64_t)s.x | ((uint64_t)s.y << 32);
      if (sk == key) return make_uint2(s.z, s.w);
      any_empty |= sk == MFX_EMPTY;
    }
    if (any_empty) break;
  }
  return make_uint2(0u, 0u);
}

__device__ __forceinline__ uint2 mfx_c_find_lean(const mfx_table_view &c, uint64_t fkey, uint32_t lineA, uint32_t d0, bool &beyond) {
  mfx_probe pr;
  pr.lineA = lineA;
  pr.lineB = c.quot ? 0u : mfx_range32(mfx_hash64(fkey), c.nlines);
  pr.b0 = 0u;
  pr.fkey = fkey;
  beyond = false;
  const uint32_t dmax = mfx_c_maxlines(c);
  for (uint32_t d = d0; d < dmax; ++d) {
    const uint4 *ln = reinterpret_cast<const uint4 *>(reinterpret_cast<const unsigned long long *>(c.slots) + mfx_probe_line(c, pr, d) * MFX_CSLOTS_LINE);
    const uint64_t key = mfx_c_keyat(c, fkey, d);
    bool any_empty = false;
#pragma unroll 1
    for (uint32_t q = 0; q < MFX_CSLOTS_LINE / 2; ++q) {
      const uint4 s = ln[q];
      const uint64_t x = (uint64_t)s.x | ((uint64_t)s.y << 32), y = (uint64_t)s.z | ((uint64_t)s.w << 32);
      if (x != MFX_EMPTY && (x >> 22) == key) return make_uint2(1u, s.x);
      if (y != MFX_EMPTY && (y >> 22) == key) return make_uint2(1u, s.z);
      any_empty |= (x == MFX_EMPTY) || (y == MFX_EMPTY);
    }
    if (any_empty) return make_uint2(0u, 0u);
  }
  beyond = c.quot != 0;
  return make_uint2(0u, 0u);
}

__device__ __forceinline__ uint2 mfx_c_fields_lean(const mfx_table_view &c, uint64_t key, uint32_t lo) {
  uint32_t rv = (lo >> 11) & MFX_CSAT, av = lo & MFX_CSAT;
  if (rv == MFX_CSAT || av == MFX_CSAT) {
    const uint2 x = mfx_side_lookup_lean(c, key);
    if (rv == MFX_CSAT) rv = x.x;
    if (av == MFX_CSAT) av = x.y;
  }
  if (rv < c.minV || rv > c.maxV) rv = 0;
  return make_uint2(rv, av);
}


__device__ __forceinline__ unsigned long long *mfx_c_claim(const mfx_table_view &c, uint64_t key, uint64_t *meta, uint32_t &fresh,
                                                           unsigned long long &cur, uint32_t init, bool &claimed, mfx_slot *&side_slot) {
  const mfx_probe pr = mfx_home(c, key);
  unsigned long long *cs = reinterpret_cast<unsigned long long *>(c.slots);
  claimed = false;
  side_slot = nullptr;
  const uint32_t q0 = 2u * pr.b0;
  const uint32_t dmax = mfx_c_maxlines(c);
  for (uint32_t d = 0; d < dmax; ++d) {
    unsigned long long *base = cs + mfx_probe_line(c, pr, d) * MFX_CSLOTS_LINE;
    const uint64_t kf = mfx_c_keyat(c, pr.fkey, d);
    const unsigned long long mine = ((unsigned long long)kf << 22) | init;
    for (uint32_t qi = 0; qi < MFX_CSLOTS_LINE; qi += 2) {
      const uint32_t q = (q0 + qi) & (MFX_CSLOTS_LINE - 1u);
      const uint4 s = *reinterpret_cast<const uint4 *>(base + q);
      const unsigned long long seen[2] = {(unsigned long long)s.x | ((unsigned long long)s.y << 32),
                                          (unsigned long long)s.z | ((unsigned long long)s.w << 32)};
#pragma unroll
      for (uint32_t e = 0; e < 2; ++e) {
        cur = seen[e];
        if (cur == MFX_EMPTY) {
          cur = atomicCAS(base + q + e, (unsigned long long)MFX_EMPTY, mine);
          if (cur == MFX_EMPTY) { ++fresh; cur = mine; claimed = true; return base + q + e; }
        }
        if ((cur >> 22) == kf) return base + q + e;
      }
    }
  }
  if (c.quot) {
    side_slot = mfx_claim(mfx_side_view(c), key, meta, fresh);
    return nullptr;
  }
  atomicAdd((unsigned long long *)&meta[2], 1ull);
  return nullptr;
}

__device__ __forceinline__ void mfx_c_add(const mfx_table_view &c, unsigned long long *w, unsigned long long cur, uint64_t key, uint32_t v,
                                          int side, uint64_t *meta) {
  if (v == 0u) return;
  const int sh = side ? 0 : 11;
  uint32_t amount;
  while (true) {
    const uint32_t f = (uint32_t)(cur >> sh) & MFX_CSAT;
    if (f == MFX_CSAT) { amount = v; break; }
    const uint64_t sum = (uint64_t)f + v;
    const unsigned long long nw = sum >= MFX_CSAT ? (cur | ((unsigned long long)MFX_CSAT << sh)) : cur + ((unsigned long long)v << sh);
    const unsigned long long old = atomicCAS(w, cur, nw);
    if (old == cur) {
      if (sum < MFX_CSAT) return;
      amount = (uint32_t)sum;
      break;
    }
    cur = old;
  }
  uint32_t side_fresh = 0;
  mfx_slot *sl = mfx_claim(mfx_side_view(c), key, meta, side_fresh);
  if (sl) atomicAdd(side ? &sl->asmV : &sl->readV, amount);
}

template <int S>
__device__ __forceinline__ uint32_t mfx_group_bcast(uint32_t v);

__device__ __forceinline__ unsigned long long mfx_slot_key_load(const mfx_table_view &t, uint32_t line, uint32_t sub) {
  return __hip_atomic_load(reinterpret_cast<unsigned long long *>(&t.slots[(uint64_t)line * MFX_SLOTS_LINE + sub].key), __ATOMIC_RELAXED,
                           __HIP_MEMORY_SCOPE_AGENT);
// ... 772 lines not shown
  for (int j = 0; j < B; ++j) {
    if (st[j] != 0xfeu) continue;
    if (dbg) atomicAdd(&dbg[2], 1ull);
    const uint64_t sk = (uint64_t)sv[j].x | ((uint64_t)sv[j].y << 32);
    if (sk == km[j] || sk == MFX_EMPTY) {
      const bool hit = sk == km[j];
      const uint2 x = mfx_sat_fill(rv[j], hit ? sv[j].z : 0u, hit ? sv[j].w : 0u);
      rv[j] = (x.x < c.minV || x.x > c.maxV) ? 0u : x.x;
      av[j] = x.y;
      st[j] = 0xffu;
    }
  }
  bool more = false;
#pragma unroll
  for (int j = 0; j < B; ++j) more |= st[j] == 0xfeu;
  if (!__any(more)) return;
#pragma unroll
  for (int j = 0; j < B; ++j)
    if (st[j] == 0xfeu) sv[j] = *reinterpret_cast<const uint4 *>(c.side + (uint64_t)mfx_range32(mfx_hash64(km[j]), c.side_nlines) * MFX_SLOTS_LINE + 1);
#pragma unroll
  for (int j = 0; j < B; ++j) {
    if (st[j] != 0xfeu) continue;
    const uint64_t sk = (uint64_t)sv[j].x | ((uint64_t)sv[j].y << 32);
    if (sk == km[j] || sk == MFX_EMPTY) {
      const bool hit = sk == km[j];
      const uint2 x = mfx_sat_fill(rv[j], hit ? sv[j].z : 0u, hit ? sv[j].w : 0u);
      rv[j] = (x.x < c.minV || x.x > c.maxV) ? 0u : x.x;
      av[j] = x.y;
      st[j] = 0xffu;
    }
  }
}

template <class F>
struct mfx_push_fn {
  static constexpr bool enabled = true;
  F f;
  __device__ __forceinline__ bool operator()(int j, bool want, uint64_t kmer, uint32_t aux, uint32_t mode) const { return f(j, want, kmer, aux, mode); }
};
struct mfx_no_push {
  static constexpr bool enabled = false;
  __device__ __forceinline__ bool operator()(int, bool, uint64_t, uint32_t, uint32_t) const { return false; }
};

#ifndef MFX_V_TAIL_STEPS
#define MFX_V_TAIL_STEPS 0
#endif
#ifndef MFX_V_BUCKET2
#define MFX_V_BUCKET2 1
#endif

template <int B, bool B2>
__device__ __forceinline__ void mfx_lane_front(const mfx_table_view &c, const uint64_t (&fkey)[B], const bool (&ok)[B], uint32_t (&rv)[B], uint32_t (&av)[B],
                                               const uint32_t (&line)[B], const uint32_t (&b0)[B], uint32_t (&st)[B], unsigned long long *dbg) {
  const uint4 *const slots0 = reinterpret_cast<const uint4 *>(c.slots);
  constexpr uint32_t HIT = 3u;
  uint4 v[B];
#pragma unroll
  for (int j = 0; j < B; ++j) v[j] = slots0[((uint64_t)line[j] << 3) | b0[j]];
  auto match = [&](int j) {
    const uint4 s = v[j];
    const uint64_t ks = fkey[j] << 22;
    const uint32_t klo = (uint32_t)ks, khi = (uint32_t)(ks >> 32);
    const bool ha = s.y == khi && ((s.x ^ klo) >> 22) == 0u, hb = s.w == khi && ((s.z ^ klo) >> 22) == 0u;
    const bool room = s.y == 0xffffffffu || s.w == 0xffffffffu;
    rv[j] = ha ? s.x : s.z;
    st[j] = (ha || hb) ? HIT : (room ? 0xffu : 1u);
  };
#pragma unroll
  for (int j = 0; j < B; ++j) {
    match(j);
    if (!ok[j]) st[j] = 0xffu;
  }
  bool left = false;
#pragma unroll
  for (int j = 0; j < B; ++j) left |= st[j] == 1u;
  if ((B2 || dbg) && __any(left)) {
    if (dbg) {
#pragma unroll
      for (int j = 0; j < B; ++j) if (st[j] == 1u) atomicAdd(&dbg[0], 1ull);
    }
    if (B2) {
#pragma unroll
      for (int j = 0; j < B; ++j)
        if (st[j] == 1u) v[j] = slots0[((uint64_t)line[j] << 3) | ((b0[j] + 1u) & 7u)];
#pragma unroll
      for (int j = 0; j < B; ++j)
        if (st[j] == 1u) {
          match(j);
          if (dbg && st[j] != 1u) atomicAdd(&dbg[6], 1ull);
        }
    }
  }
#pragma unroll
  for (int j = 0; j < B; ++j) {
    const bool found = st[j] == HIT;
    const uint32_t lo = rv[j];
    const uint32_t r_rv = (lo >> 11) & MFX_CSAT, r_av = lo & MFX_CSAT;
    const bool sat = r_rv == MFX_CSAT || r_av == MFX_CSAT;
    const uint32_t f_rv = (r_rv < c.minV || r_rv > c.maxV) ? 0u : r_rv;
    rv[j] = found ? (sat ? lo : f_rv) : 0u;
    av[j] = (found && !sat) ? r_av : 0u;
    if (found) st[j] = sat ? 0xfeu : 0xffu;
  }
}
template <int B, class KeyOf, class Push = mfx_no_push, uint32_t CAP = 64u, bool B2 = false>
__device__ __forceinline__ uint32_t mfx_lane_lookup8(const mfx_table_view &c, mfx_mailbox &M, const uint64_t (&fkey)[B], const bool (&ok)[B],
                                                     uint32_t (&rv)[B], uint32_t (&av)[B], const uint32_t (&line)[B], const uint32_t (&b0)[B],
                                                     KeyOf keyof, unsigned long long *dbg = nullptr, Push push = Push()) {
  const uint32_t tid = threadIdx.x, sub16 = (tid & 7u) << 4, lane = tid & 63u, wbase = tid & ~63u;
  uint32_t st[B];
  mfx_lane_front<B, B2>(c, fkey, ok, rv, av, line, b0, st, dbg);
#if !MFX_V_SIDE_LATE
  mfx_side_direct<B>(c, st, rv, av, keyof, dbg);
#endif
  bool left = false;
#pragma unroll
  for (int j = 0; j < B; ++j) left |= st[j] == 1u;
  if (__any(left)) {
    uint32_t qpos[B];
    uint32_t nq = 0;
#pragma unroll
    for (int j = 0; j < B; ++j) {
      const bool p = st[j] == 1u;
      const uint64_t m = __ballot(p);
      const uint32_t pos = nq + (uint32_t)__popcll(m & ((1ULL << lane) - 1ULL));
      qpos[j] = 0xffffffffu;
      if (p && pos < CAP) {
        qpos[j] = pos;
        const uint64_t ks = fkey[j] << 22;
        M.rec[wbase + pos] = make_uint4((uint32_t)ks, (uint32_t)(ks >> 32), line[j], 0u);
      }
      nq += (uint32_t)__popcll(m);
    }
    mfx_wave_handoff();
    if (nq > CAP) nq = CAP;
    constexpr uint32_t MFX_TAIL_STEPS = MFX_V_TAIL_STEPS ? MFX_V_TAIL_STEPS : (B <= 2 ? 2 : 4);
    auto tail_pass = [&](bool second) {
      for (uint32_t q0 = 0; q0 < nq; q0 += 8u * MFX_TAIL_STEPS) {
        uint4 sl[MFX_TAIL_STEPS];
        bool act[MFX_TAIL_STEPS];
#pragma unroll
        for (uint32_t sp = 0; sp < MFX_TAIL_STEPS; ++sp) {
          const uint32_t e = q0 + 8u * sp + (lane >> 3);
          sl[sp] = make_uint4(0u, 0u, 0u, 0u);
          act[sp] = false;
          if (e < nq) {
            const uint2 lw = *reinterpret_cast<const uint2 *>(reinterpret_cast<const uint32_t *>(&M.rec[wbase + e]) + 2);
            act[sp] = !second || lw.y == 2u;
            if (act[sp]) sl[sp] = *reinterpret_cast<const uint4 *>(reinterpret_cast<uint64_t>(c.slots) + ((uint64_t)lw.x << 7) + sub16);
          }
        }
        mfx_wave_handoff();
#pragma unroll
        for (uint32_t sp = 0; sp < MFX_TAIL_STEPS; ++sp) {
          const uint32_t e = q0 + 8u * sp + (lane >> 3);
          if (act[sp]) {
            uint32_t *rec = reinterpret_cast<uint32_t *>(&M.rec[wbase + e]);
            const uint2 kk = *reinterpret_cast<const uint2 *>(rec);
            if (sl[sp].y == 0xffffffffu || sl[sp].w == 0xffffffffu) rec[3] = 1u;
            if (sl[sp].y == kk.y && ((sl[sp].x ^ kk.x) >> 22) == 0u) { rec[0] = sl[sp].x; rec[2] = 0xffffffffu; }
            else if (sl[sp].w == kk.y && ((sl[sp].z ^ kk.x) >> 22) == 0u) { rec[0] = sl[sp].z; rec[2] = 0xffffffffu; }
          }
        }
      }
// ... 403 lines not shown
#endif
constexpr int MFX_BATCH = MFX_V_BATCH;

#ifndef MFX_V_MINBLOCKS
#define MFX_V_MINBLOCKS 4
#endif
#ifndef MFX_V_MINBLOCKS_K21
#define MFX_V_MINBLOCKS_K21 7
#endif
#ifndef MFX_V_BATCH_K21
#define MFX_V_BATCH_K21 2
#endif
#ifndef MFX_V_MINBLOCKS_K31
#define MFX_V_MINBLOCKS_K31 6
#endif
#ifndef MFX_V_BATCH_K31
#define MFX_V_BATCH_K31 2
#endif
#ifndef MFX_V_MINBLOCKS_GEN
#define MFX_V_MINBLOCKS_GEN 4
#endif
#ifndef MFX_V_BATCH_GEN
#define MFX_V_BATCH_GEN 4
#endif
#ifndef MFX_V_DEFER_K21
#define MFX_V_DEFER_K21 0
#endif
#ifndef MFX_V_DEFER_K31
#define MFX_V_DEFER_K31 1
#endif
#ifndef MFX_V_KFXLDS_K21
#define MFX_V_KFXLDS_K21 1
#endif
constexpr uint32_t MFX_KFX_BASE = 32u;
#ifndef MFX_V_BUCKET2_K21
#define MFX_V_BUCKET2_K21 0
#endif
#ifndef MFX_V_BUCKET2_K31
#define MFX_V_BUCKET2_K31 1
#endif
template <bool CANON, bool COMPACT, int KF> struct mfx_hist_tune { static constexpr int blocks = MFX_V_MINBLOCKS, batch = MFX_V_BATCH, defer = 0, kfxlds = 0, bucket2 = 0; };
template <> struct mfx_hist_tune<true, true, 21> { static constexpr int blocks = MFX_V_MINBLOCKS_K21, batch = MFX_V_BATCH_K21, defer = MFX_V_DEFER_K21, kfxlds = MFX_V_KFXLDS_K21, bucket2 = MFX_V_BUCKET2_K21; };
#ifndef MFX_V_KFXLDS_K31
#define MFX_V_KFXLDS_K31 0
#endif
template <> struct mfx_hist_tune<true, true, 31> { static constexpr int blocks = MFX_V_MINBLOCKS_K31, batch = MFX_V_BATCH_K31, defer = MFX_V_DEFER_K31, kfxlds = MFX_V_KFXLDS_K31, bucket2 = MFX_V_BUCKET2_K31; };
template <> struct mfx_hist_tune<true, true, 0> { static constexpr int blocks = MFX_V_MINBLOCKS_GEN, batch = MFX_V_BATCH_GEN, defer = 0, kfxlds = 0, bucket2 = 0; };
template <int BT>
__device__ __forceinline__ uint32_t mfx_hist_cell(uint32_t wv, uint32_t j) { return wv * (uint32_t)BT + j; }
template <int BT>
__device__ __forceinline__ uint32_t mfx_hist_pos(uint32_t b, uint32_t wv, uint32_t tid, uint32_t j) { return b * MFX_BLOCK + (mfx_hist_cell<BT>(wv, j) << 6) + (tid & 63u); }
template <int BT>
__device__ __forceinline__ uint32_t mfx_hist_slot(uint32_t wv, uint32_t j) { return mfx_hist_cell<BT>(wv, j) & (MFX_BLOCK / 64 - 1u); }
template <bool CANON, bool COMPACT, int KF, int WF, int TF, bool DBG = false>
__global__ __launch_bounds__(MFX_BLOCK, (mfx_hist_tune<CANON, COMPACT, KF>::blocks)) void mfx_hist_kernel(mfx_hist_args a) {
  constexpr int BT = mfx_hist_tune<CANON, COMPACT, KF>::batch;
  __shared__ mfx_tile_lds L;
  __shared__ mfx_mailbox MB;
  __shared__ mfx_hist_lds H;

  const uint32_t tid = threadIdx.x;
  const uint32_t wv = (uint32_t)__builtin_amdgcn_readfirstlane((int)(tid >> 6));
  if (KF) { a.t.k = KF; a.t.mz_w = WF; a.t.mz_t = TF; a.t.quot = KF > MFX_MAX_K_DIRECT ? 1 : 0; }
  const int k = KF ? KF : a.t.k;
  const mfx_kstar_args &ka = a.ks;
  mfx_hist_lds_init(H, ka);
  const bool lut_ok = H.lut_ok != 0u;

  uint32_t n_valid = 0, n_missing = 0, n_over0 = 0;
  if (tid == 0) { H.tot[0] = H.tot[1] = 0; H.wl_n = 0u; }
  if (tid < MFX_BLOCK / 64) H.kfx_slot[tid] = 0ull;
  uint64_t *c_glob = ka.counts + 2ull * ka.nbins;
  uint64_t *c_kasm = c_glob + 3, *c_kmis = c_kasm + ka.ncontigs;

  const uint32_t none = 0xffffffffu;
  uint32_t c = none;
  uint64_t li = blockIdx.x;
  for (uint32_t it = 0; li < a.n_logical; ++it) {
    if (tid == 0)
      H.next[it & 1] = (uint64_t)gridDim.x + atomicAdd((unsigned long long *)a.tile_ctr, 1ull);
    const uint64_t tile = a.part_n == 1 ? a.tile_begin + li
                                         : ((((li >> a.part_shift) * a.part_n + a.part_rank) << a.part_shift) | (li & ((1ull << a.part_shift) - 1ull)));
    const uint32_t cn = a.tile_contig[tile];
    if (cn != c) {
      if (c != none) {
        uint64_t x = n_valid, y = n_missing, z = 0;
        mfx_block_sum3(x, y, z, H.red);
        if (tid == 0 && (x | y)) {
          atomicAdd((unsigned long long *)&c_kasm[c], x);
          atomicAdd((unsigned long long *)&c_kmis[c], y);
          H.tot[0] += x;
          H.tot[1] += y;
        }
        n_valid = n_missing = 0;
      }
      c = cn;
    }
    const uint64_t pos0 = (tile - a.tile_start[c]) * MFX_TILE;
    const uint64_t clen = a.contig_len[c];
    const uint32_t n = (clen - pos0 < MFX_TILE) ? (uint32_t)(clen - pos0) : MFX_TILE;
    const uint8_t *src = a.bases + a.contig_off[c] + pos0;

    if (a.codes) {
      const uint64_t w0 = (a.contig_off[c] + pos0) >> 5;
      mfx_tile_fill_packed(L, a.codes + w0, a.valid + w0);
    } else {
      mfx_tile_fill(L, src);
    }
    __syncthreads();

    constexpr bool kfx_lds = mfx_hist_tune<CANON, COMPACT, KF>::kfxlds != 0 && COMPACT && CANON && KF != 0 && TF != 0;
    constexpr uint32_t mb_cap = kfx_lds ? MFX_KFX_BASE : 64u;
    static_assert(!(mfx_hist_tune<CANON, COMPACT, KF>::kfxlds != 0 && mfx_hist_tune<CANON, COMPACT, KF>::defer != 0),
                  "kfxlds keeps a count of at most 16 in 8 bits of one LDS word per lane: the deferred probe lets a lane evaluate more than its own 16 k-mers of a tile");
    static_assert(MFX_TILE / MFX_BLOCK <= 16, "the lane's word (an 8-bit count of the dominant bin) holds 16 evaluations per lane and tile");
    static_assert(MFX_TILE / (MFX_BLOCK / 64) <= 1024, "a slot's word holds the terms (at most 2^52 units each) of 1024 positions of a tile");
    unsigned long long *const kfxw = reinterpret_cast<unsigned long long *>(&MB.rec[(tid & ~63u) + MFX_KFX_BASE]) + (tid & 63u);
    if (kfx_lds) *kfxw = 0ull;
    struct lds_bump { unsigned long long *w; __device__ __forceinline__ void operator++(int) { (void)__hip_atomic_fetch_add(reinterpret_cast<uint32_t *>(w) + 1, 1u << 24, __ATOMIC_RELAXED, __HIP_MEMORY_SCOPE_WORKGROUP); } };
    struct lds_sum { unsigned long long *w; __device__ __forceinline__ void operator+=(uint64_t v) { (void)__hip_atomic_fetch_add(w, (unsigned long long)v, __ATOMIC_RELAXED, __HIP_MEMORY_SCOPE_WORKGROUP); } };
    auto eval1 = [&](uint32_t rvv, uint32_t avv, uint32_t slot) {
      lds_sum sum{&H.kfx_slot[slot]};
      if (kfx_lds) {
        lds_bump bump{kfxw};
        if (mfx_hist_eval_fx(H, ka, lut_ok, rvv, avv, bump, sum)) n_missing++;
      } else if (mfx_hist_eval_fx(H, ka, lut_ok, rvv, avv, n_over0, sum)) n_missing++;
    };
    const bool wave_lines = COMPACT && CANON && (KF ? TF != 0 : a.t.mz_t != 0);
    const bool defer_tail = MFX_V_DEFER != 0 && mfx_hist_tune<CANON, COMPACT, KF>::defer != 0 && COMPACT && CANON && KF != 0 && TF != 0 && (KF & 1) != 0;
    const bool quotf = KF ? KF > MFX_MAX_K_DIRECT : a.t.quot != 0;
    constexpr bool bucket2 = MFX_V_BUCKET2 != 0 && mfx_hist_tune<CANON, COMPACT, KF>::bucket2 != 0;
    auto push_wave = [&](bool want, uint64_t kmer, uint32_t aux, uint32_t mode, bool dbl, uint32_t slot) -> bool {
      if (!a.wl) return false;
      const uint64_t m = __ballot(want);
      if (!m) return false;
      const uint32_t ln = tid & 63u, leader = (uint32_t)__ffsll((unsigned long long)m) - 1u;
      uint32_t base = 0;
      if (ln == leader) base = atomicAdd(&H.wl_n, (uint32_t)__popcll(m));
      base = (uint32_t)__shfl((int)base, (int)leader, 64);
      const uint32_t at = base + (uint32_t)__popcll(m & ((1ULL << ln) - 1ULL));
      const bool fits = want && at < a.wl_segcap;
      if (fits) reinterpret_cast<uint4 *>(a.wl + MFX_WL_HEADER)[(uint64_t)blockIdx.x * a.wl_segcap + at] =
                  make_uint4((uint32_t)kmer, (uint32_t)(kmer >> 32), aux, ((uint32_t)li * (MFX_BLOCK / 64) + slot) | (dbl ? 0x80000000u : 0u) | (mode << 29));
      return fits;
    };
    uint32_t nq = 0;
    uint32_t *const mwave = reinterpret_cast<uint32_t *>(H.dred) + (tid >> 6) * 128u;
    for (uint32_t b = 0;; b += BT) {
      const bool last = b >= MFX_TILE / MFX_BLOCK || b * MFX_BLOCK >= n;
      nq = (uint32_t)__builtin_amdgcn_readfirstlane((int)nq);
      if (defer_tail && (last || nq >= (MFX_DEFER_FLUSH < mb_cap ? MFX_DEFER_FLUSH : mb_cap / 2u))) {
        auto kmer_at = [&](uint32_t p) -> uint64_t {
          uint64_t f;
          (void)mfx_tile_kmer(L, k, p, f);
          const uint64_t r = mfx_revcomp(f, k);
          return f < r ? f : r;
        };
        auto eval_at = [&](uint32_t rvv, uint32_t avv, uint32_t p) { eval1(rvv, avv, (p >> 6) & (MFX_BLOCK / 64 - 1u)); };
        mfx_lane_flush(a.t, MB, nq, kmer_at, eval_at, [&](bool want, uint64_t km, uint32_t aux, uint32_t mode, uint32_t p) { return push_wave(want, km, aux, mode, false, (p >> 6) & (MFX_BLOCK / 64 - 1u)); }, DBG ? reinterpret_cast<unsigned long long *>(a.dbg) : nullptr);
      }
      if (last) break;
      uint32_t rv[BT], av[BT];
      bool     ok[BT];
      uint32_t parked = 0u;
      const bool even_k = KF ? (KF & 1) == 0 : (k & 1) == 0;
      if (wave_lines) {
        uint64_t fkey[BT];
        uint32_t line[BT], b0[BT];
        uint32_t halo[2], pal = 0u;
        mfx_wave_mod_halo<BT>(a.t, L, mfx_hist_pos<BT>(b, wv, tid, 0u), 64u, halo);
#pragma unroll
        for (int j = 0; j < BT; ++j) {
          const uint32_t p = mfx_hist_pos<BT>(b, wv, tid, (uint32_t)j);
          uint64_t f;
          ok[j] = mfx_tile_kmer(L, k, p, f) && (p < n);
          const uint64_t r = mfx_revcomp(f, k);
          line[j] = mfx_wave_mod_line(a.t, mwave, halo, j, f, r, b0[j], fkey[j]);
          if (!ok[j]) { line[j] = 0u; b0[j] = 0u; }
          if (even_k && f == r) pal |= 1u << j;
        }
        const bool quot = quotf;
        auto keyof = [&](int sj) -> uint64_t {
          uint64_t kk = 0;
          if (!quot) {
#pragma unroll
            for (int j = 0; j < BT; ++j) if (j == sj) kk = fkey[j];
          } else {
            uint64_t f;
            (void)mfx_tile_kmer(L, k, mfx_hist_pos<BT>(b, wv, tid, (uint32_t)sj), f);
            const uint64_t r = mfx_revcomp(f, k);
            kk = f < r ? f : r;
          }
          return kk;
        };
        if (defer_tail) {
          uint32_t posn[BT];
#pragma unroll
          for (int j = 0; j < BT; ++j) posn[j] = mfx_hist_pos<BT>(b, wv, tid, (uint32_t)j);
          auto pj = [&](int jj, bool want, uint64_t km, uint32_t aux, uint32_t mode) { return push_wave(want, km, aux, mode, false, mfx_hist_slot<BT>(wv, (uint32_t)jj)); };
          parked = mfx_lane_probe_defer<BT, decltype(keyof), mfx_push_fn<decltype(pj)>, mb_cap, bucket2>(
                       a.t, MB, nq, fkey, ok, rv, av, line, b0, posn, keyof, DBG ? reinterpret_cast<unsigned long long *>(a.dbg) : nullptr, mfx_push_fn<decltype(pj)>{pj});
        } else {
          auto pj = [&](int jj, bool want, uint64_t km, uint32_t aux, uint32_t mode) { return push_wave(want, km, aux, mode, ((pal >> jj) & 1u) != 0u, mfx_hist_slot<BT>(wv, (uint32_t)jj)); };
          parked = mfx_lane_lookup8<BT, decltype(keyof), mfx_push_fn<decltype(pj)>, mb_cap, bucket2>(
                       a.t, MB, fkey, ok, rv, av, line, b0, keyof, DBG ? reinterpret_cast<unsigned long long *>(a.dbg) : nullptr, mfx_push_fn<decltype(pj)>{pj});
        }
        if (even_k) {
#pragma unroll
          for (int j = 0; j < BT; ++j) if ((pal >> j) & 1u) { rv[j] += rv[j]; av[j] += av[j]; }
        }
      } else {
        uint64_t key[BT], key2[BT];
#pragma unroll
        for (int j = 0; j < BT; ++j) {
          const uint32_t p = mfx_hist_pos<BT>(b, wv, tid, (uint32_t)j);
          uint64_t f;
          ok[j] = mfx_tile_kmer(L, k, p, f) && (p < n);
          const uint64_t r = mfx_revcomp(f, k);
          if (CANON) {
            key[j] = f < r ? f : r; key2[j] = f < r ? r : f;
          } else {
            key[j] = f; key2[j] = r;
          }
        }
        if (COMPACT) mfx_compact_lookup<BT>(a.t, MB, key, key2, ok, rv, av);
        else mfx_group_lookup<BT>(a.t, MB, key, key2, ok, rv, av);
        if (!CANON) {
          uint32_t rv2[BT], av2[BT];
          if (COMPACT) mfx_compact_lookup<BT>(a.t, MB, key2, key, ok, rv2, av2);
          else mfx_group_lookup<BT>(a.t, MB, key2, key, ok, rv2, av2);
#pragma unroll
          for (int j = 0; j < BT; ++j) { rv[j] += rv2[j]; av[j] += av2[j]; }
        } else if (even_k) {
#pragma unroll
          for (int j = 0; j < BT; ++j) if (key[j] == key2[j]) { rv[j] += rv[j]; av[j] += av[j]; }
        }
      }
#pragma unroll
      for (int j = 0; j < BT; ++j) {
        if (!ok[j]) continue;
        n_valid++;
        if (!((parked >> j) & 1u)) eval1(rv[j], av[j], mfx_hist_slot<BT>(wv, (uint32_t)j));
      }
    }
    if (kfx_lds) { mfx_wave_handoff(); n_over0 += (uint32_t)(*kfxw >> 56); }

    __syncthreads();
    if (tid < MFX_BLOCK / 64) {
      reinterpret_cast<uint64_t *>(a.tile_partials)[li * (MFX_BLOCK / 64) + tid] = H.kfx_slot[tid];
      H.kfx_slot[tid] = 0ull;
    }
    const uint64_t nx = H.next[it & 1];
    li = ((uint64_t)__builtin_amdgcn_readfirstlane((uint32_t)(nx >> 32)) << 32) |
         (uint64_t)__builtin_amdgcn_readfirstlane((uint32_t)nx);
  }
  {
    uint64_t x = n_valid, y = n_missing, z = n_over0;
    mfx_block_sum3(x, y, z, H.red);
// ... 1086 lines not shown
  __shared__ mfx_tile_lds L;
  const uint32_t tid = threadIdx.x;
  const int k = a.t.k;
  uint32_t fresh = 0;
  for (uint64_t tile = blockIdx.x; tile < a.ntiles; tile += gridDim.x) {
    uint32_t lo = 0, hi = a.ncontigs;
    while (hi - lo > 1) {
      uint32_t mid = lo + (hi - lo) / 2;
      if (a.tile_start[mid] <= tile) lo = mid; else hi = mid;
    }
    uint32_t c = lo;
    const uint64_t pos0 = (tile - a.tile_start[c]) * MFX_TILE;
    const uint64_t clen = a.contig_len[c];
    const uint32_t n = (clen - pos0 < MFX_TILE) ? (uint32_t)(clen - pos0) : MFX_TILE;
    __syncthreads();
    if (a.codes) {
      const uint64_t w0 = (a.contig_off[c] + pos0) >> 5;
      mfx_tile_fill_packed(L, a.codes + w0, a.valid + w0);
    } else {
      mfx_tile_fill(L, a.bases + a.contig_off[c] + pos0);
    }
    __syncthreads();
    for (uint32_t b = 0; b < MFX_TILE / MFX_BLOCK; ++b) {
      if (b * MFX_BLOCK >= n) break;
      uint32_t p = b * MFX_BLOCK + tid;
      uint64_t f;
      bool ok = mfx_tile_kmer(L, k, p, f) && p < n;
      const uint64_t r = mfx_revcomp(f, k);
      const uint64_t key = f < r ? f : r;
      if (ok && a.t.shard_n > 1 && mfx_owner(a.t, key, f < r ? r : f, a.t.shard_n) != a.t.shard_rank) ok = false;
      if (a.count == 2) {
        if (a.t.compact) {
          if (ok) {
            const mfx_probe pr = mfx_home(a.t, key);
            unsigned long long *mb = reinterpret_cast<unsigned long long *>(a.t.slots) + mfx_probe_line(a.t, pr, 0) * MFX_CSLOTS_LINE + 2u * pr.b0;
            const uint4 s4 = *reinterpret_cast<const uint4 *>(mb);
            const uint64_t x = (uint64_t)s4.x | ((uint64_t)s4.y << 32), y = (uint64_t)s4.z | ((uint64_t)s4.w << 32);
            unsigned long long *w = nullptr;
            unsigned long long cur = 0;
            bool beyond = false;
            if (x == MFX_EMPTY) { }
            else if ((x >> 22) == pr.fkey) { w = mb; cur = x; }
            else if (y == MFX_EMPTY) { }
            else if ((y >> 22) == pr.fkey) { w = mb + 1; cur = y; }
            else w = mfx_c_find(a.t, pr, 0, cur, beyond);
            if (w) mfx_c_add(a.t, w, cur, key, 1u, 1, a.meta);
            else if (beyond) { mfx_slot *ss = mfx_find_slot(mfx_side_view(a.t), key); if (ss) atomicAdd(&ss->asmV, 1u); }
          }
        } else {
          uint32_t dropped = 0;
          mfx_group_insert<false>(a.t, key, ok ? 1u : 0u, 1, a.meta, dropped);
        }
      } else if (a.t.compact) {
        if (ok) {
          unsigned long long cur = 0;
          bool claimed;
          mfx_slot *ss;
          unsigned long long *w = mfx_c_claim(a.t, key, a.meta, fresh, cur, a.count ? 1u : 0u, claimed, ss);
          if (w && a.count && !claimed) mfx_c_add(a.t, w, cur, key, 1u, 1, a.meta);
          else if (ss && a.count) atomicAdd(&ss->asmV, 1u);
        }
      } else if (MODE == 1 && a.count) mfx_group_insert(a.t, key, ok ? 1u : 0u, 1, a.meta, fresh);
      else if (ok) {
        mfx_slot *sl = mfx_claim(a.t, key, a.meta, fresh);
        if (sl && a.count) atomicAdd(&sl->asmV, 1u);
      }
    }
  }
  mfx_meta_flush(a.meta, fresh, 0u);
}


__device__ __forceinline__ bool mfx_c_add_read(const mfx_table_view &c, unsigned long long *w, unsigned long long cur, uint64_t key, uint32_t v,
                                               uint64_t *meta) {
  uint32_t amount;
  bool moved = false;
  while (true) {
    const uint32_t f = (uint32_t)(cur >> 11) & MFX_CSAT;
    if (f == MFX_CSAT) { amount = v; break; }
    const uint64_t sum = (uint64_t)f + v;
    const unsigned long long nw = sum >= MFX_CSAT ? (cur | ((unsigned long long)MFX_CSAT << 11)) : cur + ((unsigned long long)v << 11);
    const unsigned long long old = atomicCAS(w, cur, nw);
    if (old == cur) {
      if (sum < MFX_CSAT) return false;
      amount = (uint32_t)sum;
      moved = true;
      break;
    }
    cur = old;
  }
  uint32_t side_fresh = 0;
  mfx_slot *sl = mfx_claim(mfx_side_view(c), key, meta, side_fresh);
  if (sl) atomicAdd(&sl->readV, amount);
  return moved;
}

__device__ __forceinline__ mfx_slot *mfx_reads_find16(const mfx_table_view &t, uint64_t key) {
  const mfx_probe pr = mfx_home(t, key);
  for (uint32_t d = 0; d < MFX_MAX_LINES; ++d) {
    mfx_slot *ln = t.slots + mfx_probe_line(t, pr, d) * MFX_SLOTS_LINE;
    bool any_empty = false;
#pragma unroll 1
    for (uint32_t q = 0; q < MFX_SLOTS_LINE; ++q) {
      const uint4 s = *reinterpret_cast<const uint4 *>(ln + q);
      const uint64_t sk = (uint64_t)s.x | ((uint64_t)s.y << 32);
      if (sk == key) return ln + q;
      any_empty |= sk == MFX_EMPTY;
    }
    if (any_empty) break;
  }
  return nullptr;
}

// ... 323 lines not shown
  const char *me = getenv("MFX_INSERT_MODE");
  const int mode = me ? atoi(me) : 1;
  if (mode == 0)      mfx_table_add_kernel<0><<<(unsigned)blocks, 256, 0, st>>>(t, kmers, values, n, side, meta);
  else                mfx_table_add_kernel<1><<<(unsigned)blocks, 256, 0, st>>>(t, kmers, values, n, side, meta);
  return hipGetLastError();
}
static uint32_t mfx_ingest_grid(uint32_t nblocks) {
  uint32_t cap = 8192u;
  if (const char *e = getenv("MFX_INGEST_GRID")) { const long v = atol(e); if (v >= 1 && v <= 8192) cap = (uint32_t)v; }
  return nblocks < cap ? nblocks : cap;
}
hipError_t mfx_k_table_add_delta(mfx_table_view t, const uint64_t *payload, const uint64_t *dir, uint32_t nblocks, uint64_t n,
                                 uint64_t payload_base, int side, uint64_t *meta, hipStream_t st) {
  if (nblocks == 0) return hipSuccess;
  mfx_table_add_delta_kernel<<<mfx_ingest_grid(nblocks), 256, 0, st>>>(t, payload, dir, nblocks, n, payload_base, side, meta);
  return hipGetLastError();
}
int mfx_k_table_takes_placed(const mfx_table_view &t) {
#if MFX_V_PLACE_OLDLINE || MFX_V_PLACE_WBUCKET
  if (!t.quot) return 0;
#endif
  return t.compact && t.seq_only && t.k >= MFX_PLACE_MIN_K && t.k <= MFX_PLACE_MAX_K && t.mz_w == MFX_PLACE_W && t.mz_t == mfx_p_tlen(t.k) && t.shard_n <= 1;
}
hipError_t mfx_k_table_add_placed(mfx_table_view t, const uint64_t *payload, const uint64_t *dir, uint32_t nblocks, uint64_t n,
                                  uint64_t payload_base, int side, uint64_t *meta, hipStream_t st) {
  if (nblocks == 0) return hipSuccess;
  mfx_table_add_placed_kernel<<<mfx_ingest_grid(nblocks), 256, 0, st>>>(t, payload, dir, nblocks, n, payload_base, side, meta, mfx_k_table_takes_placed(t));
  return hipGetLastError();
}
hipError_t mfx_k_place_keys(int k, const uint64_t *kmers, uint64_t n, uint64_t *out, hipStream_t st) {
  if (n == 0) return hipSuccess;
  uint64_t blocks = (n + 255) / 256;
  if (blocks > 8192) blocks = 8192;
  mfx_place_keys_kernel<<<(unsigned)blocks, 256, 0, st>>>(k, kmers, n, out);
  return hipGetLastError();
}
hipError_t mfx_k_table_value(mfx_table_view t, const uint64_t *kmers, uint64_t n, uint32_t *readV, uint32_t *asmV,
                             hipStream_t st) {
  if (n == 0) return hipSuccess;
  uint64_t blocks = (n + 255) / 256;
  if (blocks > 8192) blocks = 8192;
  mfx_table_value_kernel<<<(unsigned)blocks, 256, 0, st>>>(t, kmers, n, readV, asmV);
  return hipGetLastError();
}
hipError_t mfx_k_table_export(mfx_table_view t, uint64_t *kmers, uint32_t *readV, uint32_t *asmV,
                              unsigned long long *count, hipStream_t st) {
  mfx_table_export_kernel<<<4096, 256, 0, st>>>(t, kmers, readV, asmV, count);
  return hipGetLastError();
}
hipError_t mfx_k_hist(const mfx_hist_args &a, int grid, hipStream_t st) {
  static const unsigned dyn = getenv("MFX_DEBUG_DYN_LDS") ? (unsigned)atoi(getenv("MFX_DEBUG_DYN_LDS")) : 0u;
  const char *ge = getenv("MFX_HIST_GENERIC");
  const bool generic = ge && atoi(ge);
  if (a.dbg && a.canonical && a.t.compact && a.t.k == 21 && a.t.mz_w == 4 && a.t.mz_t == 6 && !generic) mfx_hist_kernel<true, true, 21, 4, 6, true><<<grid, MFX_BLOCK, dyn, st>>>(a);
  else if (a.canonical && a.t.compact && a.t.k == 21 && a.t.mz_w == 4 && a.t.mz_t == 6 && !generic) mfx_hist_kernel<true, true, 21, 4, 6><<<grid, MFX_BLOCK, dyn, st>>>(a);
  else if (a.canonical && a.t.compact && a.t.k == 21 && a.t.mz_w == 5 && a.t.mz_t == 7 && !generic) mfx_hist_kernel<true, true, 21, 5, 7><<<grid, MFX_BLOCK, dyn, st>>>(a);
  else if (a.dbg && a.canonical && a.t.compact && a.t.quot && a.t.k == 31 && a.t.mz_w == 4 && a.t.mz_t == 4 && !generic) mfx_hist_kernel<true, true, 31, 4, 4, true><<<grid, MFX_BLOCK, dyn, st>>>(a);
  else if (a.canonical && a.t.compact && a.t.quot && a.t.k == 31 && a.t.mz_w == 4 && a.t.mz_t == 4 && !generic) mfx_hist_kernel<true, true, 31, 4, 4><<<grid, MFX_BLOCK, dyn, st>>>(a);
  else if (a.canonical && a.t.compact) mfx_hist_kernel<true, true, 0, 0, 0><<<grid, MFX_BLOCK, dyn, st>>>(a);
  else if (a.canonical)                mfx_hist_kernel<true, false, 0, 0, 0><<<grid, MFX_BLOCK, dyn, st>>>(a);
  else if (a.t.compact)                mfx_hist_kernel<false, true, 0, 0, 0><<<grid, MFX_BLOCK, dyn, st>>>(a);
  else                                 mfx_hist_kernel<false, false, 0, 0, 0><<<grid, MFX_BLOCK, dyn, st>>>(a);
  return hipGetLastError();
}
hipError_t mfx_k_hist_rest(const mfx_hist_args &a, int grid, hipStream_t st) {
  if (!a.wl) return hipSuccess;
  mfx_hist_rest_kernel<<<grid, MFX_BLOCK, 0, st>>>(a);
  return hipGetLastError();
}
hipError_t mfx_k_route(const mfx_route_args &a, hipStream_t st) {
  uint64_t nt = a.tile_end - a.tile_begin;
  if (nt == 0) return hipSuccess;
  mfx_route_kernel<<<(unsigned)(nt < 4096 ? nt : 4096), MFX_BLOCK, 0, st>>>(a);
  return hipGetLastError();
}
hipError_t mfx_k_route_split(const mfx_route_args &a, uint64_t *keys_out, uint32_t *contig_out, hipStream_t st) {
  const uint64_t nt = a.tile_end - a.tile_begin;
  if (nt == 0) return hipSuccess;
  const unsigned grid = (unsigned)(nt < 4096 ? nt : 4096);
  mfx_route_count_kernel<<<grid, MFX_BLOCK, 0, st>>>(a);
  mfx_route_scan_kernel<<<a.nranks, MFX_BLOCK, 0, st>>>(a.tile_cnt, nt, a.nranks, a.dest_counts);
  mfx_route_scatter_kernel<<<grid, MFX_BLOCK, 0, st>>>(a, keys_out, contig_out);
  return hipGetLastError();
}
hipError_t mfx_k_route_gather(const mfx_route_args &a, const uint32_t *idx, uint64_t nvalid, uint64_t *keys_out,
                              uint32_t *contig_out, hipStream_t st) {
  if (nvalid == 0) return hipSuccess;
  mfx_route_gather_kernel<<<2048, 256, 0, st>>>(a, idx, nvalid, keys_out, contig_out);
  return hipGetLastError();
}
hipError_t mfx_k_iota(uint32_t *v, uint64_t n, hipStream_t st) {
  if (n == 0) return hipSuccess;
  mfx_iota_kernel<<<2048, 256, 0, st>>>(v, n);
  return hipGetLastError();
}
hipError_t mfx_k_hist_keys(const mfx_hist_keys_args &a, int grid, hipStream_t st) {
  if (a.nseg) mfx_hist_keys_kernel<true><<<grid, MFX_BLOCK, 0, st>>>(a);
  else        mfx_hist_keys_kernel<false><<<grid, MFX_BLOCK, 0, st>>>(a);
  return hipGetLastError();
}
hipError_t mfx_k_route_fused(const mfx_route_args &a, uint64_t *keys_out, uint32_t *contig_out, uint64_t *cursors, uint64_t region_cap, hipStream_t st) {
  const uint64_t nt = a.tile_end - a.tile_begin;
  if (nt == 0) return hipSuccess;
  mfx_route_fused_kernel<<<(unsigned)(nt < 4096 ? nt : 4096), MFX_BLOCK, 0, st>>>(a, keys_out, contig_out, reinterpret_cast<unsigned long long *>(cursors), region_cap);
  return hipGetLastError();
}
hipError_t mfx_k_sum_partials(const double *partials, uint32_t n, double *out, hipStream_t st) {
// ... 165 lines not shown
```

merfin_amd/csrc/mfx_reads.cpp:

```cpp
#include "mfx_internal.h"
#include "mfx_kernels.h"
#include "mfx_grow.h"
#include "mfx_bin.h"

#include <chrono>

#include <string.h>

#include <algorithm>
#include <vector>

extern "C" void mfx_pack_bases(const uint8_t *src, uint64_t n, uint64_t *codes, uint32_t *valid);

namespace {
constexpr uint64_t MFX_READS_BATCH_DEFAULT = MFX_BATCH_BASES_DEFAULT;
constexpr int MFX_READS_STAGES = 2;
constexpr uint64_t MFX_TILE_WORDS_HOST = (MFX_TILE + 64) / 32;

struct DeviceScope {
  int prev = -1;
  bool ok = false;
  explicit DeviceScope(int dev) {
    if (hipGetDevice(&prev) != hipSuccess) prev = -1;
    ok = hipSetDevice(dev) == hipSuccess;
// ... 108 lines not shown
  mfx_slot *ns = nullptr;
  uint64_t *nmeta = nullptr;
  MFX_HIP(hipMalloc((void **)&nmeta, MFX_META_WORDS * sizeof(uint64_t)));
  while (true) {
    const uint64_t new_bytes = new_lines * MFX_ALIGN;
    size_t free_b = 0, total_b = 0;
    const bool known = hipMemGetInfo(&free_b, &total_b) == hipSuccess;
    if (!known) (void)hipGetLastError();
    if ((ix->max_gb > 0 && (double)old_bytes + (double)new_bytes > ix->max_gb * 1e9) || (known && new_bytes > free_b) ||
        hipMalloc((void **)&ns, new_bytes) != hipSuccess) {
      (void)hipGetLastError();
      (void)hipFree(nmeta);
      return mfx_fail(MFX_E_NOMEM, "the k-mer table cannot grow from %.6f GB to %.6f GB (%lu k-mers stored): both tables are held while the entries move, "
                      "under a limit of %.6f GB (-memory; 0: none) with %.6f GB of device memory free", (double)old_bytes / 1e9, (double)new_bytes / 1e9,
                      (unsigned long)distinct, ix->max_gb, known ? (double)free_b / 1e9 : 0.0);
    }
    mfx_table_view nt = ix->view();
    nt.slots = ns;
    nt.nlines = new_lines;
    nt.qshift = 0;
    for (uint64_t x = new_lines; x > 1; x >>= 1) ++nt.qshift;
    hipEvent_t e0 = nullptr, e1 = nullptr;
    uint64_t meta[MFX_META_WORDS] = {0};
    float ms = 0;
    const bool ok = mfx_memset_now(nmeta, 0, MFX_META_WORDS * sizeof(uint64_t)) == hipSuccess && hipEventCreate(&e0) == hipSuccess &&
                    hipEventCreate(&e1) == hipSuccess && mfx_k_table_init(ns, new_lines * MFX_SLOTS_LINE, nullptr) == hipSuccess &&
                    hipEventRecord(e0, nullptr) == hipSuccess &&
                    mfx_k_table_rehash(ix->d_slots, ix->nlines * MFX_SLOTS_LINE, nt, nmeta, nullptr) == hipSuccess &&
                    hipEventRecord(e1, nullptr) == hipSuccess && hipEventSynchronize(e1) == hipSuccess &&
                    hipEventElapsedTime(&ms, e0, e1) == hipSuccess &&
                    hipMemcpy(meta, nmeta, sizeof(meta), hipMemcpyDeviceToHost) == hipSuccess;
    const hipError_t err = ok ? hipSuccess : hipGetLastError();
    if (e0) (void)hipEventDestroy(e0);
    if (e1) (void)hipEventDestroy(e1);
    if (!ok) {
      (void)hipFree(ns);
      (void)hipFree(nmeta);
      return mfx_fail(MFX_E_HIP, "moving the k-mer table into a larger one failed: %s", hipGetErrorString(err));
    }
    ix->rehash_seconds += ms * 1e-3;
    ix->rehash_bytes += old_bytes + meta[0] * 2 * MFX_ALIGN;
    if (meta[2] == 0 && meta[0] == distinct) break;
    (void)hipFree(ns);
    ns = nullptr;
    if (meta[2] == 0) {
      (void)hipFree(nmeta);
      return mfx_fail(MFX_E_HIP, "moving the k-mer table into a larger one lost entries: %lu of %lu arrived", (unsigned long)meta[0], (unsigned long)distinct);
    }
    if (new_lines > ((1ull << 32) - 16) / 2) { (void)hipFree(nmeta); return mfx_fail(MFX_E_NOMEM, "the k-mer table cannot grow beyond 2^32 lines (%.6f GB now, %.6f GB tried)", (double)old_bytes / 1e9, (double)new_bytes / 1e9); }
    new_lines *= 2;
  }
  (void)hipFree(nmeta);
  (void)hipFree(ix->d_slots);
  ix->d_slots = ns;
  ix->nlines = new_lines;
  ix->capacity_kmers = (uint64_t)((double)new_lines * MFX_SLOTS_LINE * 0.7);
  ix->version++;
  return MFX_OK;
}

static int claim_reserve(mfx_reads *r, uint64_t B) {
  mfx_index *ix = r->ix;
#ifdef MFX_V_GROW_NO_PENDING
  const uint64_t pending = 0;
#else
  const uint64_t pending = r->pending;
#endif
  if (mfx_grow_fits(r->distinct_known, pending, B, ix->nlines * MFX_SLOTS_LINE)) return MFX_OK;
  for (auto &s : r->S) if (int rc = stage_settle(r, s)) return rc;
  uint64_t meta[3] = {0, 0, 0};
  MFX_HIP(hipMemcpy(meta, ix->d_meta, sizeof(meta), hipMemcpyDeviceToHost));
  r->distinct_known = meta[0];
  r->pending = 0;
  if (mfx_grow_fits(r->distinct_known, 0, B, ix->nlines * MFX_SLOTS_LINE)) return MFX_OK;
  const uint64_t nl = mfx_grow_lines(r->distinct_known, B, ix->nlines, MFX_SLOTS_LINE, (1ull << 32) - 16);
  if (nl == 0)
    return mfx_fail(MFX_E_NOMEM, "the k-mer table cannot grow from %.6f GB to one that holds %lu k-mers and a batch of %lu positions: beyond 2^32 lines "
                    "(%.6f GB)", (double)ix->nlines * MFX_ALIGN / 1e9, (unsigned long)r->distinct_known, (unsigned long)B, (double)(1ull << 32) * MFX_ALIGN / 1e9);
  const auto t0 = std::chrono::steady_clock::now();
  const int rc = table_grow(ix, nl, r->distinct_known);
  if (rc == MFX_OK) {
    ix->grow_count += 1;
    ix->grow_seconds += std::chrono::duration<double>(std::chrono::steady_clock::now() - t0).count();
  }
  return rc;
}

template <class Fill>
static int reads_send(mfx_reads *r, uint64_t npos, Fill &&fill) {
  if (npos == 0) return MFX_OK;
  mfx_reads::Stage &s = r->S[r->cur];
  if (int rc = stage_settle(r, s)) return rc;
  if (r->claim) {
    if (int rc = claim_reserve(r, npos)) {
      r->fail_code = rc;
      r->fail_text = mfx_last_error();
      return rc;
    }
    r->pending += npos;
  }
  const uint64_t ntiles = (npos + MFX_TILE - 1) / MFX_TILE;
  const uint64_t nw = std::min(r->words, ntiles * (MFX_TILE / 32) + MFX_TILE_WORDS_HOST);
  fill(s.hc, s.hv, nw);
  mfx_reads_args a;
  a.t = r->ix->view();
  a.codes = s.dc;
// ... 277 lines not shown
```

merfin_amd/csrc/mfx_stream_plan.h:

```cpp
#pragma once
#include "mfx_internal.h"

#include <string.h>
#include <algorithm>
#include <vector>

extern "C" void mfx_pack_bases(const uint8_t *src, uint64_t n, uint64_t *codes, uint32_t *valid);

inline void seq_layout_fill(mfx_seq *s, const uint64_t *lens, uint32_t ncontigs) {
  s->ncontigs = ncontigs;
  s->off.resize(ncontigs);
  s->len.assign(lens, lens + ncontigs);
  s->tile_start.resize((size_t)ncontigs + 1);
  uint64_t o = 0, t = 0;
  for (uint32_t c = 0; c < ncontigs; ++c) {
    s->off[c] = o;
    s->tile_start[c] = t;
    t += (lens[c] + MFX_TILE - 1) / MFX_TILE;
    s->total_bases += lens[c];
    o = (o + lens[c] + 1 + MFX_ALIGN - 1) / MFX_ALIGN * MFX_ALIGN;
  }
  s->tile_start[ncontigs] = t;
  s->ntiles = t;
  s->buf_bytes = o + MFX_TILE + 2 * MFX_ALIGN;
}

struct Piece { uint32_t contig; uint64_t pos, n; };

inline void chunk_pieces(const mfx_seq *s, uint64_t t0, uint64_t t1, std::vector<Piece> &out) {
  out.clear();
  uint32_t c = (uint32_t)(std::upper_bound(s->tile_start.begin(), s->tile_start.end(), t0) - s->tile_start.begin()) - 1;
  for (; c < s->ncontigs && s->tile_start[c] < t1; ++c) {
    const uint64_t cb = std::max(t0, s->tile_start[c]), ce = std::min(t1, s->tile_start[c + 1]);
    if (ce <= cb) continue;
    const uint64_t p0 = (cb - s->tile_start[c]) * MFX_TILE;
    const uint64_t p1 = std::min<uint64_t>(s->len[c], (ce - s->tile_start[c]) * MFX_TILE + MFX_ALIGN);
    if (p1 > p0) out.push_back({c, p0, p1 - p0});
  }
}

inline std::vector<uint64_t> stream_cuts(uint64_t T, uint64_t CH0, uint64_t CH) {
  std::vector<uint64_t> cuts, tail;
  uint64_t back = 0;
  for (uint64_t sz = 2 * CH0; sz < CH && back + sz + CH <= T / 2; sz *= 2) { tail.push_back(sz); back += sz; }
  const uint64_t front_end = T - back;
  uint64_t t0 = 0;
  for (uint64_t sz = CH0; t0 < front_end; sz = std::min(CH, sz * 2)) {
    uint64_t t1 = std::min(front_end, t0 + sz);
    if (front_end - t1 < sz / 2) t1 = front_end;
    cuts.push_back(t1);
    t0 = t1;
  }
  for (size_t i = tail.size(); i-- > 0;) { t0 += tail[i]; cuts.push_back(t0); }
  return cuts;
}
inline std::vector<uint64_t> upload_cuts(uint64_t T, uint64_t CH) {
  std::vector<uint64_t> cuts;
  for (uint64_t t0 = 0; t0 < T; t0 += CH) cuts.push_back(std::min(T, t0 + CH));
  return cuts;
}

struct StreamChunk { std::vector<Piece> pieces; uint64_t lo = 0, hi = 0, t0 = 0, t1 = 0; };

// ... 55 lines not shown
```

Baseline: 158.2 billion.

## Record per-position slot hints at index build and use them in hist lookups

While the seq-only compact k=21 index is being counted, a 4-bit hint per sequence position is stored in a device plane. The hint records whether the k-mer landed in its first probe line and which slot pair it occupies. The hist kernel then reads these hints to jump straight to the recorded bucket and to skip the 'room' early-exit on hinted positions, with the aim of cutting extra slot scans and second-bucket probes. This costs an extra device plane of half a byte per base plus one byte load per k-mer. Correctness relies on the sequence layout hash matching between build and evaluation.

```diff
diff --git a/include/merfin_amd.h b/include/merfin_amd.h
--- a/include/merfin_amd.h
+++ b/include/merfin_amd.h
@@ -226,6 +226,8 @@
 int       mfx_eval_debug_worklist(mfx_eval *ev, int mode, uint32_t segcap);
 int       mfx_eval_debug_worklist_read(mfx_eval *ev, int slot, uint32_t *segs, uint32_t *segcap, uint64_t *counts, uint64_t counts_cap,
                                        void *entries, uint64_t entries_cap, uint64_t *n_entries);
+
+int       mfx_index_debug_hints(mfx_index *ix, int op, uint8_t *buf, uint64_t buf_bytes, uint64_t *bytes);
 
 int mfx_debug_traverse_host(const void *clusters, uint64_t ncl, const void *variants, uint64_t nvar, const void *alleles, uint64_t nal,
                             const char *win_text, uint64_t win_bytes, const char *al_text, uint64_t al_bytes, uint64_t text_end,
diff --git a/merfin_amd/binding.py b/merfin_amd/binding.py
--- a/merfin_amd/binding.py
+++ b/merfin_amd/binding.py
@@ -79,7 +79,7 @@
     "mfx_seq_upload", "mfx_seq_from_device", "mfx_seq_free", "mfx_seq_num_contigs", "mfx_seq_num_bases",
     "mfx_seq_num_tiles", "mfx_seq_is_packed",
     "mfx_diag_gather_rate",
-    "mfx_eval_create", "mfx_eval_free", "mfx_eval_nbins", "mfx_eval_debug_enable", "mfx_eval_debug_counters", "mfx_eval_debug_worklist", "mfx_eval_debug_worklist_read", "mfx_getK", "mfx_getKmetric", "mfx_histoQV",
+    "mfx_eval_create", "mfx_eval_free", "mfx_eval_nbins", "mfx_eval_debug_enable", "mfx_eval_debug_counters", "mfx_eval_debug_worklist", "mfx_eval_debug_worklist_read", "mfx_index_debug_hints", "mfx_getK", "mfx_getKmetric", "mfx_histoQV",
     "mfx_hist_run", "mfx_hist_result_free", "mfx_hist_launch", "mfx_hist_launch_cyclic", "mfx_hist_result_from_counts",
     "mfx_hist_take_overflow", "mfx_hist_report", "mfx_diag_stream_rates",
     "mfx_pack_bases", "mfx_host_threads_share", "mfx_dump_values", "mfx_dump_contig", "mfx_dump_values_sharded", "mfx_dump_contig_sharded", "mfx_variants_run_sharded", "mfx_vcf_load", "mfx_vcf_free", "mfx_variants_run_vcf", "mfx_vcf_prepare", "mfx_vcf_path_bound", "mfx_index_claim_paths", "mfx_vcf_prepare_path_index", "mfx_completeness", "mfx_completeness_pieces", "mfx_variants_run",
@@ -267,6 +267,7 @@
     L.mfx_eval_debug_enable.argtypes = [vp, C.c_int]
     L.mfx_eval_debug_counters.argtypes = [vp, u64p]
     L.mfx_eval_debug_worklist.argtypes = [vp, C.c_int, C.c_uint32]
+    L.mfx_index_debug_hints.argtypes = [vp, C.c_int, C.POINTER(C.c_uint8), C.c_uint64, u64p]
     L.mfx_eval_debug_worklist_read.argtypes = [vp, C.c_int, u32p, u32p, u64p, C.c_uint64, vp, C.c_uint64, u64p]
     L.mfx_getK.argtypes = [C.POINTER(_KP), C.c_uint32, C.c_uint32, f64p, f64p, f64p]
     L.mfx_getKmetric.restype = C.c_double
@@ -947,6 +948,23 @@
     def count_asm(self, seqs, stream=None):
         _check(load_library().mfx_index_count_asm(self.h, seqs.h, C.c_void_p(stream or 0)))
 
+    def debug_hints(self, op="read", plane=None):
+        L = load_library()
+        n = C.c_uint64(0)
+        u8p = C.POINTER(C.c_uint8)
+        if op == "read":
+            _check(L.mfx_index_debug_hints(self.h, 0, None, 0, C.byref(n)))
+            out = np.zeros(n.value, dtype=np.uint8)
+            if n.value:
+                _check(L.mfx_index_debug_hints(self.h, 0, out.ctypes.data_as(u8p), len(out), C.byref(n)))
+            return out
+        if op == "write":
+            plane = np.ascontiguousarray(plane, dtype=np.uint8)
+            _check(L.mfx_index_debug_hints(self.h, 3, plane.ctypes.data_as(u8p), len(plane), C.byref(n)))
+            return n.value
+        _check(L.mfx_index_debug_hints(self.h, {"drop": 1, "restore": 2}[op], None, 0, C.byref(n)))
+        return n.value
+
     def count_reads(self, reads, batch_bases=0, minV=0, maxV=2**64 - 1, chunk=4096):
         return self._count_reads(load_library().mfx_reads_begin, reads, batch_bases, minV, maxV, chunk)
 
@@ -1768,7 +1786,7 @@
         _check(load_library().mfx_eval_debug_counters(self.h, out.ctypes.data_as(C.POINTER(C.c_uint64))))
         return {"first_pass": int(out[0]), "second_pass": int(out[1]), "side_table": int(out[2]), "line_scans": int(out[3]),
                 "side_not_in_two_slots": int(out[4]), "ended_per_lane": int(out[5]),
-                "second_bucket": int(out[6])}
+                "second_bucket": int(out[6]), "hint_ended": int(out[7])}
 
     def debug_worklist(self, mode=1, segcap=0):
         _check(load_library().mfx_eval_debug_worklist(self.h, mode, segcap))
diff --git a/merfin_amd/csrc/mfx_api.cpp b/merfin_amd/csrc/mfx_api.cpp
--- a/merfin_amd/csrc/mfx_api.cpp
+++ b/merfin_amd/csrc/mfx_api.cpp
@@ -2,6 +2,7 @@
 #include "mfx_histsum.h"
 #include "mfx_place.h"
 #include "mfx_kernels.h"
+#include "mfx_hints.h"
 #include "mfx_pipe.h"
 #include "mfx_pool.h"
 #include "mfx_stream_plan.h"
@@ -367,6 +368,7 @@
   if (!ix) return;
   DevGuard g(ix->device);
   mfx_index_ingest_release(ix);
+  mfx_index_drop_hints(ix);
   if (ix->d_slots) (void)hipFree(ix->d_slots);
   if (ix->d_meta) (void)hipFree(ix->d_meta);
   delete ix;
@@ -767,6 +769,7 @@
   return index_add(ix, kmers, values, n, 1, on_device);
 }
 
+static uint8_t *index_hint_plane(mfx_index *ix, const mfx_seq *seq);
 static int index_count(mfx_index *ix, const mfx_seq *seq, int count, void *stream, const char *who, bool defer = false, bool no_wait = false) {
   if (!ix || !seq) return mfx_fail(MFX_E_INVAL, "%s: null argument", who);
   if (ix->device != seq->device) return mfx_fail(MFX_E_INVAL, "index and sequence live on different devices");
@@ -799,6 +802,7 @@
     ix->seq_digest = d;
   }
   if (count == 2) ix->frozen = true;
+  else a.hints = index_hint_plane(ix, seq);
   MFX_HIP(ix->wide() ? mfx_kw_count(a, (hipStream_t)stream) : mfx_k_count(a, (hipStream_t)stream));
   if (no_wait) return MFX_OK;
   if (defer) {
@@ -1272,6 +1276,45 @@
   return MFX_OK;
 }
 
+uint64_t mfx_seq_layout_hash(const mfx_seq *s) {
+  std::lock_guard<std::mutex> lazy(s->lazy_mu);
+  if (s->layout_hash == 0) s->layout_hash = mfx_hint_layout_hash(s->off.data(), s->len.data(), s->ncontigs);
+  return s->layout_hash;
+}
+
+void mfx_index_drop_hints(mfx_index *ix) {
+  if (!ix) return;
+  DevGuard g(ix->device);
+  if (ix->d_hints) (void)hipFree(ix->d_hints);
+  if (ix->d_hints_parked) (void)hipFree(ix->d_hints_parked);
+  ix->d_hints = ix->d_hints_parked = nullptr;
+  ix->hints_bytes = ix->hints_layout = 0;
+}
+
+static uint8_t *index_hint_plane(mfx_index *ix, const mfx_seq *seq) {
+  if (!ix->seq_only || !ix->compact || ix->quot || ix->k != 21 || ix->shard_n != 1 || ix->paths_token) return nullptr;
+  const uint64_t bytes = mfx_hint_plane_bytes(seq->buf_bytes), layout = mfx_seq_layout_hash(seq);
+  if (ix->d_hints_parked) mfx_index_drop_hints(ix);
+  if (ix->d_hints && (ix->hints_bytes != bytes || ix->hints_layout != layout)) mfx_index_drop_hints(ix);
+  if (!ix->d_hints) {
+    if (ix->max_gb > 0 && ((double)ix->total_lines() * MFX_ALIGN + (double)bytes) / 1e9 > ix->max_gb) return nullptr;
+    if (hipMalloc((void **)&ix->d_hints, bytes) != hipSuccess) {
+      (void)hipGetLastError();
+      ix->d_hints = nullptr;
+      return nullptr;
+    }
+    if (mfx_memset_now(ix->d_hints, 0, bytes) != hipSuccess) {
+      (void)hipGetLastError();
+      (void)hipFree(ix->d_hints);
+      ix->d_hints = nullptr;
+      return nullptr;
+    }
+    ix->hints_bytes = bytes;
+    ix->hints_layout = layout;
+  }
+  return ix->d_hints;
+}
+
 thread_local bool t_mfx_path_lookup = false;
 int mfx_check_seq_of_index(const mfx_index *ix, const mfx_seq *s, const char *who) {
   if (!ix->seq_only || ix->seq_digest == 0) return MFX_OK;
@@ -1675,6 +1718,10 @@
   a.ks.partials = ev->d_partials;
   a.ks.ovf = ev->d_ovf;
   a.dbg = ev->d_dbg;
+  if (ev->ix->d_hints && ev->ix->hints_bytes == mfx_hint_plane_bytes(seq->buf_bytes) && ev->ix->hints_layout == mfx_seq_layout_hash(seq)) {
+    const char *hn_env = getenv("MFX_HIST_HINTS");
+    if (!(hn_env && atoi(hn_env) == 0)) a.hints = ev->ix->d_hints;
+  }
   const char *wl_env = getenv("MFX_HIST_WORKLIST");
   const bool wl_off = (wl_env && atoi(wl_env) == 0) || ev->dbg_wl_mode == 0;
   ev->wl_used_segs[ctr_slot] = ev->wl_used_segcap[ctr_slot] = 0;
diff --git a/merfin_amd/csrc/mfx_debug.cpp b/merfin_amd/csrc/mfx_debug.cpp
--- a/merfin_amd/csrc/mfx_debug.cpp
+++ b/merfin_amd/csrc/mfx_debug.cpp
@@ -176,3 +176,29 @@
   }
   return MFX_OK;
 }
+
+extern "C" int mfx_index_debug_hints(mfx_index *ix, int op, uint8_t *buf, uint64_t buf_bytes, uint64_t *bytes) {
+  if (!ix) return mfx_fail(MFX_E_INVAL, "mfx_index_debug_hints: null argument");
+  if (op < 0 || op > 3) return mfx_fail(MFX_E_INVAL, "mfx_index_debug_hints: op %d (0 read, 1 drop, 2 restore, 3 overwrite)", op);
+  int prev = 0;
+  MFX_HIP(hipGetDevice(&prev));
+  MFX_HIP(hipSetDevice(ix->device));
+  struct Back { int d; ~Back() { (void)hipSetDevice(d); } } back{prev};
+  MFX_HIP(hipDeviceSynchronize());
+  if (op == 1) {
+    if (ix->d_hints) { ix->d_hints_parked = ix->d_hints; ix->d_hints = nullptr; }
+  } else if (op == 2) {
+    if (ix->d_hints_parked) { ix->d_hints = ix->d_hints_parked; ix->d_hints_parked = nullptr; }
+  } else if (op == 3) {
+    if (!ix->d_hints) return mfx_fail(MFX_E_INVAL, "mfx_index_debug_hints: the index has no hint plane to overwrite");
+    if (!buf || buf_bytes != ix->hints_bytes)
+      return mfx_fail(MFX_E_INVAL, "mfx_index_debug_hints: the plane has %lu bytes, the caller's array %lu", (unsigned long)ix->hints_bytes, (unsigned long)buf_bytes);
+    MFX_HIP(hipMemcpy(ix->d_hints, buf, buf_bytes, hipMemcpyHostToDevice));
+  } else if (buf && ix->d_hints) {
+    if (buf_bytes < ix->hints_bytes)
+      return mfx_fail(MFX_E_INVAL, "mfx_index_debug_hints: the plane has %lu bytes, the caller's buffer holds %lu", (unsigned long)ix->hints_bytes, (unsigned long)buf_bytes);
+    MFX_HIP(hipMemcpy(buf, ix->d_hints, ix->hints_bytes, hipMemcpyDeviceToHost));
+  }
+  if (bytes) *bytes = ix->d_hints ? ix->hints_bytes : 0;
+  return MFX_OK;
+}
diff --git a/merfin_amd/csrc/mfx_hints.h b/merfin_amd/csrc/mfx_hints.h
--- /dev/null
+++ b/merfin_amd/csrc/mfx_hints.h
@@ -0,0 +1,36 @@
+#pragma once
+#include <stddef.h>
+#include <stdint.h>
+
+#if defined(__HIPCC__) || defined(__CUDACC__)
+#define MFX_HINT_FN __host__ __device__ inline
+#else
+#define MFX_HINT_FN inline
+#endif
+
+constexpr uint32_t MFX_HINT_SET = 8u;
+
+MFX_HINT_FN uint64_t mfx_hint_plane_bytes(uint64_t buf_bytes) { return (buf_bytes + 1) / 2; }
+MFX_HINT_FN uint64_t mfx_hint_byte(uint64_t g) { return g >> 1; }
+MFX_HINT_FN uint32_t mfx_hint_shift(uint64_t g) { return (uint32_t)(g & 1u) << 2; }
+MFX_HINT_FN uint32_t mfx_hint_get(const uint8_t *plane, uint64_t g) { return ((uint32_t)plane[mfx_hint_byte(g)] >> mfx_hint_shift(g)) & 15u; }
+MFX_HINT_FN uint8_t mfx_hint_pair(uint32_t even_nibble, uint32_t odd_nibble) { return (uint8_t)((even_nibble & 15u) | ((odd_nibble & 15u) << 4)); }
+MFX_HINT_FN uint32_t mfx_hint_of_slot(uint32_t cand, uint32_t slot_in_line) { return cand == 0u ? (MFX_HINT_SET | ((slot_in_line >> 1) & 7u)) : 0u; }
+MFX_HINT_FN uint32_t mfx_hint_bucket(uint32_t nibble, uint32_t b0) { return (nibble & MFX_HINT_SET) ? (nibble & 7u) : b0; }
+MFX_HINT_FN bool mfx_hint_is_set(uint32_t nibble) { return (nibble & MFX_HINT_SET) != 0u; }
+
+inline void mfx_hint_put(uint8_t *plane, uint64_t g, uint32_t nibble) {
+  uint8_t &b = plane[mfx_hint_byte(g)];
+  b = (uint8_t)((b & ~(15u << mfx_hint_shift(g))) | ((nibble & 15u) << mfx_hint_shift(g)));
+}
+
+inline uint64_t mfx_hint_layout_hash(const uint64_t *off, const uint64_t *len, size_t ncontigs) {
+  uint64_t h = 0x9E3779B97F4A7C15ull ^ (uint64_t)ncontigs;
+  auto mix = [&](uint64_t v) {
+    h ^= v + 0x9E3779B97F4A7C15ull + (h << 6) + (h >> 2);
+    h *= 0xD6E8FEB86659FD93ull;
+    h ^= h >> 32;
+  };
+  for (size_t c = 0; c < ncontigs; ++c) { mix(off[c]); mix(len[c]); }
+  return h ? h : 1ull;
+}
diff --git a/merfin_amd/csrc/mfx_internal.h b/merfin_amd/csrc/mfx_internal.h
--- a/merfin_amd/csrc/mfx_internal.h
+++ b/merfin_amd/csrc/mfx_internal.h
@@ -138,6 +138,9 @@
   uint64_t  side_nlines = 0;
   uint64_t  paths_token = 0;
   uint32_t  seq_digest = 0;
+  uint8_t  *d_hints = nullptr;
+  uint8_t  *d_hints_parked = nullptr;
+  uint64_t  hints_bytes = 0, hints_layout = 0;
   double    max_gb = 0;
   uint64_t  grow_count = 0, rehash_bytes = 0;
   double    grow_seconds = 0, rehash_seconds = 0;
@@ -168,6 +171,7 @@
   uint64_t  part_lo = 0, part_hi = 0;
   mutable std::mutex lazy_mu;
   mutable uint32_t digest = 0;
+  mutable uint64_t layout_hash = 0;
 };
 
 template <class Alloc, class Release, class Fill>
@@ -189,6 +193,8 @@
 }
 
 int mfx_seq_digest32(const mfx_seq *s, uint32_t *out);
+uint64_t mfx_seq_layout_hash(const mfx_seq *s);
+void mfx_index_drop_hints(mfx_index *ix);
 int mfx_check_seq_of_index(const mfx_index *ix, const mfx_seq *s, const char *who);
 extern thread_local bool t_mfx_path_lookup;
 
diff --git a/merfin_amd/csrc/mfx_kernels.h b/merfin_amd/csrc/mfx_kernels.h
--- a/merfin_amd/csrc/mfx_kernels.h
+++ b/merfin_amd/csrc/mfx_kernels.h
@@ -32,6 +32,7 @@
   uint64_t       *dbg = nullptr;
   uint64_t       *wl = nullptr;
   uint32_t        wl_segs = 0, wl_segcap = 0;
+  const uint8_t  *hints = nullptr;
   mfx_kstar_args  ks;
 };
 
@@ -157,6 +158,7 @@
   uint64_t        ntiles;
   uint64_t       *meta;
   int             count = 1;
+  uint8_t        *hints = nullptr;
 };
 
 struct mfx_reads_args {
diff --git a/merfin_amd/csrc/mfx_kernels.hip b/merfin_amd/csrc/mfx_kernels.hip
--- a/merfin_amd/csrc/mfx_kernels.hip
+++ b/merfin_amd/csrc/mfx_kernels.hip
@@ -1,6 +1,7 @@
 #include "mfx_internal.h"
 #include "mfx_kernels.h"
 #include "mfx_device.h"
+#include "mfx_hints.h"
 #include "mfx_place.h"
 #include "mfx_track.h"
 #define MFX_REGIONS_DEVICE
@@ -411,17 +412,19 @@
 
 
 __device__ __forceinline__ unsigned long long *mfx_c_claim(const mfx_table_view &c, uint64_t key, uint64_t *meta, uint32_t &fresh,
-                                                           unsigned long long &cur, uint32_t init, bool &claimed, mfx_slot *&side_slot) {
+                                                           unsigned long long &cur, uint32_t init, bool &claimed, mfx_slot *&side_slot, uint32_t &cand) {
   const mfx_probe pr = mfx_home(c, key);
   unsigned long long *cs = reinterpret_cast<unsigned long long *>(c.slots);
   claimed = false;
   side_slot = nullptr;
+  cand = 0u;
   const uint32_t q0 = 2u * pr.b0;
   const uint32_t dmax = mfx_c_maxlines(c);
   for (uint32_t d = 0; d < dmax; ++d) {
     unsigned long long *base = cs + mfx_probe_line(c, pr, d) * MFX_CSLOTS_LINE;
     const uint64_t kf = mfx_c_keyat(c, pr.fkey, d);
     const unsigned long long mine = ((unsigned long long)kf << 22) | init;
+    cand = d;
     for (uint32_t qi = 0; qi < MFX_CSLOTS_LINE; qi += 2) {
       const uint32_t q = (q0 + qi) & (MFX_CSLOTS_LINE - 1u);
       const uint4 s = *reinterpret_cast<const uint4 *>(base + q);
@@ -1300,7 +1303,7 @@
 
 template <int B, bool B2>
 __device__ __forceinline__ void mfx_lane_front(const mfx_table_view &c, const uint64_t (&fkey)[B], const bool (&ok)[B], uint32_t (&rv)[B], uint32_t (&av)[B],
-                                               const uint32_t (&line)[B], const uint32_t (&b0)[B], uint32_t (&st)[B], unsigned long long *dbg) {
+                                               const uint32_t (&line)[B], const uint32_t (&b0)[B], uint32_t (&st)[B], unsigned long long *dbg, uint32_t hinted = 0u, uint32_t moved = 0u) {
   const uint4 *const slots0 = reinterpret_cast<const uint4 *>(c.slots);
   constexpr uint32_t HIT = 3u;
   uint4 v[B];
@@ -1311,7 +1314,7 @@
     const uint64_t ks = fkey[j] << 22;
     const uint32_t klo = (uint32_t)ks, khi = (uint32_t)(ks >> 32);
     const bool ha = s.y == khi && ((s.x ^ klo) >> 22) == 0u, hb = s.w == khi && ((s.z ^ klo) >> 22) == 0u;
-    const bool room = s.y == 0xffffffffu || s.w == 0xffffffffu;
+    const bool room = (s.y == 0xffffffffu || s.w == 0xffffffffu) && !((hinted >> j) & 1u);
     rv[j] = ha ? s.x : s.z;
     st[j] = (ha || hb) ? HIT : (room ? 0xffu : 1u);
   };
@@ -1319,6 +1322,11 @@
   for (int j = 0; j < B; ++j) {
     match(j);
     if (!ok[j]) st[j] = 0xffu;
+  }
+  if (dbg && moved) {
+#pragma unroll
+    for (int j = 0; j < B; ++j)
+      if (((moved >> j) & 1u) && st[j] != 1u) { atomicAdd(&dbg[0], 1ull); atomicAdd(&dbg[7], 1ull); }
   }
   bool left = false;
 #pragma unroll
@@ -1355,10 +1363,10 @@
 template <int B, class KeyOf, class Push = mfx_no_push, uint32_t CAP = 64u, bool B2 = false>
 __device__ __forceinline__ uint32_t mfx_lane_lookup8(const mfx_table_view &c, mfx_mailbox &M, const uint64_t (&fkey)[B], const bool (&ok)[B],
                                                      uint32_t (&rv)[B], uint32_t (&av)[B], const uint32_t (&line)[B], const uint32_t (&b0)[B],
-                                                     KeyOf keyof, unsigned long long *dbg = nullptr, Push push = Push()) {
+                                                     KeyOf keyof, unsigned long long *dbg = nullptr, Push push = Push(), uint32_t hinted = 0u, uint32_t moved = 0u) {
   const uint32_t tid = threadIdx.x, sub16 = (tid & 7u) << 4, lane = tid & 63u, wbase = tid & ~63u;
   uint32_t st[B];
-  mfx_lane_front<B, B2>(c, fkey, ok, rv, av, line, b0, st, dbg);
+  mfx_lane_front<B, B2>(c, fkey, ok, rv, av, line, b0, st, dbg, hinted, moved);
 #if !MFX_V_SIDE_LATE
   mfx_side_direct<B>(c, st, rv, av, keyof, dbg);
 #endif
@@ -1868,8 +1876,9 @@
 __device__ __forceinline__ uint32_t mfx_hist_pos(uint32_t b, uint32_t wv, uint32_t tid, uint32_t j) { return b * MFX_BLOCK + (mfx_hist_cell<BT>(wv, j) << 6) + (tid & 63u); }
 template <int BT>
 __device__ __forceinline__ uint32_t mfx_hist_slot(uint32_t wv, uint32_t j) { return mfx_hist_cell<BT>(wv, j) & (MFX_BLOCK / 64 - 1u); }
-template <bool CANON, bool COMPACT, int KF, int WF, int TF, bool DBG = false>
+template <bool CANON, bool COMPACT, int KF, int WF, int TF, bool DBG = false, bool HINTS = false>
 __global__ __launch_bounds__(MFX_BLOCK, (mfx_hist_tune<CANON, COMPACT, KF>::blocks)) void mfx_hist_kernel(mfx_hist_args a) {
+  static_assert(!HINTS || (CANON && COMPACT && KF != 0 && KF <= MFX_MAX_K_DIRECT && TF != 0), "hints are read by the direct-form instances of a fixed k");
   constexpr int BT = mfx_hist_tune<CANON, COMPACT, KF>::batch;
   __shared__ mfx_tile_lds L;
   __shared__ mfx_mailbox MB;
@@ -1960,6 +1969,7 @@
                   make_uint4((uint32_t)kmer, (uint32_t)(kmer >> 32), aux, ((uint32_t)li * (MFX_BLOCK / 64) + slot) | (dbl ? 0x80000000u : 0u) | (mode << 29));
       return fits;
     };
+    const uint8_t *const hint_tile = HINTS ? a.hints + mfx_hint_byte(a.contig_off[c] + pos0) : nullptr;
     uint32_t nq = 0;
     uint32_t *const mwave = reinterpret_cast<uint32_t *>(H.dred) + (tid >> 6) * 128u;
     for (uint32_t b = 0;; b += BT) {
@@ -1984,6 +1994,14 @@
         uint64_t fkey[BT];
         uint32_t line[BT], b0[BT];
         uint32_t halo[2], pal = 0u;
+        uint32_t hbyte[BT], hinted = 0u, moved = 0u;
+        if (HINTS) {
+#pragma unroll
+          for (int j = 0; j < BT; ++j) {
+            const uint32_t p = mfx_hist_pos<BT>(b, wv, tid, (uint32_t)j);
+            hbyte[j] = p < n ? (uint32_t)hint_tile[p >> 1] : 0u;
+          }
+        }
         mfx_wave_mod_halo<BT>(a.t, L, mfx_hist_pos<BT>(b, wv, tid, 0u), 64u, halo);
 #pragma unroll
         for (int j = 0; j < BT; ++j) {
@@ -1994,6 +2012,14 @@
           line[j] = mfx_wave_mod_line(a.t, mwave, halo, j, f, r, b0[j], fkey[j]);
           if (!ok[j]) { line[j] = 0u; b0[j] = 0u; }
           if (even_k && f == r) pal |= 1u << j;
+          if (HINTS && !defer_tail) {
+            const uint32_t nib = hbyte[j] >> ((tid & 1u) << 2);
+            if (ok[j] && mfx_hint_is_set(nib)) {
+              if (DBG && mfx_hint_bucket(nib, b0[j]) != b0[j]) moved |= 1u << j;
+              b0[j] = mfx_hint_bucket(nib, b0[j]);
+              hinted |= 1u << j;
+            }
+          }
         }
         const bool quot = quotf;
         auto keyof = [&](int sj) -> uint64_t {
@@ -2019,7 +2045,7 @@
         } else {
           auto pj = [&](int jj, bool want, uint64_t km, uint32_t aux, uint32_t mode) { return push_wave(want, km, aux, mode, ((pal >> jj) & 1u) != 0u, mfx_hist_slot<BT>(wv, (uint32_t)jj)); };
           parked = mfx_lane_lookup8<BT, decltype(keyof), mfx_push_fn<decltype(pj)>, mb_cap, bucket2>(
-                       a.t, MB, fkey, ok, rv, av, line, b0, keyof, DBG ? reinterpret_cast<unsigned long long *>(a.dbg) : nullptr, mfx_push_fn<decltype(pj)>{pj});
+                       a.t, MB, fkey, ok, rv, av, line, b0, keyof, DBG ? reinterpret_cast<unsigned long long *>(a.dbg) : nullptr, mfx_push_fn<decltype(pj)>{pj}, hinted, moved);
         }
         if (even_k) {
 #pragma unroll
@@ -3212,13 +3238,20 @@
           mfx_group_insert<false>(a.t, key, ok ? 1u : 0u, 1, a.meta, dropped);
         }
       } else if (a.t.compact) {
+        uint32_t nib = 0u;
         if (ok) {
           unsigned long long cur = 0;
           bool claimed;
           mfx_slot *ss;
-          unsigned long long *w = mfx_c_claim(a.t, key, a.meta, fresh, cur, a.count ? 1u : 0u, claimed, ss);
+          uint32_t cand;
+          unsigned long long *w = mfx_c_claim(a.t, key, a.meta, fresh, cur, a.count ? 1u : 0u, claimed, ss, cand);
+          if (w) nib = mfx_hint_of_slot(cand, (uint32_t)(w - reinterpret_cast<unsigned long long *>(a.t.slots)) & (MFX_CSLOTS_LINE - 1u));
           if (w && a.count && !claimed) mfx_c_add(a.t, w, cur, key, 1u, 1, a.meta);
           else if (ss && a.count) atomicAdd(&ss->asmV, 1u);
+        }
+        if (a.hints) {
+          const uint32_t odd = (uint32_t)__shfl_xor((int)nib, 1, 64);
+          if (!(tid & 1u) && p < n) a.hints[mfx_hint_byte(a.contig_off[c] + pos0 + p)] = mfx_hint_pair(nib, odd);
         }
       } else if (MODE == 1 && a.count) mfx_group_insert(a.t, key, ok ? 1u : 0u, 1, a.meta, fresh);
       else if (ok) {
@@ -3648,7 +3681,11 @@
   static const unsigned dyn = getenv("MFX_DEBUG_DYN_LDS") ? (unsigned)atoi(getenv("MFX_DEBUG_DYN_LDS")) : 0u;
   const char *ge = getenv("MFX_HIST_GENERIC");
   const bool generic = ge && atoi(ge);
-  if (a.dbg && a.canonical && a.t.compact && a.t.k == 21 && a.t.mz_w == 4 && a.t.mz_t == 6 && !generic) mfx_hist_kernel<true, true, 21, 4, 6, true><<<grid, MFX_BLOCK, dyn, st>>>(a);
+  const bool k21 = a.canonical && a.t.compact && !a.t.quot && a.t.k == 21 && !generic;
+  if (a.hints && a.dbg && k21 && a.t.mz_w == 4 && a.t.mz_t == 6) mfx_hist_kernel<true, true, 21, 4, 6, true, true><<<grid, MFX_BLOCK, dyn, st>>>(a);
+  else if (a.hints && k21 && a.t.mz_w == 4 && a.t.mz_t == 6) mfx_hist_kernel<true, true, 21, 4, 6, false, true><<<grid, MFX_BLOCK, dyn, st>>>(a);
+  else if (a.hints && k21 && a.t.mz_w == 5 && a.t.mz_t == 7) mfx_hist_kernel<true, true, 21, 5, 7, false, true><<<grid, MFX_BLOCK, dyn, st>>>(a);
+  else if (a.dbg && a.canonical && a.t.compact && a.t.k == 21 && a.t.mz_w == 4 && a.t.mz_t == 6 && !generic) mfx_hist_kernel<true, true, 21, 4, 6, true><<<grid, MFX_BLOCK, dyn, st>>>(a);
   else if (a.canonical && a.t.compact && a.t.k == 21 && a.t.mz_w == 4 && a.t.mz_t == 6 && !generic) mfx_hist_kernel<true, true, 21, 4, 6><<<grid, MFX_BLOCK, dyn, st>>>(a);
   else if (a.canonical && a.t.compact && a.t.k == 21 && a.t.mz_w == 5 && a.t.mz_t == 7 && !generic) mfx_hist_kernel<true, true, 21, 5, 7><<<grid, MFX_BLOCK, dyn, st>>>(a);
   else if (a.dbg && a.canonical && a.t.compact && a.t.quot && a.t.k == 31 && a.t.mz_w == 4 && a.t.mz_t == 4 && !generic) mfx_hist_kernel<true, true, 31, 4, 4, true><<<grid, MFX_BLOCK, dyn, st>>>(a);
diff --git a/merfin_amd/csrc/mfx_reads.cpp b/merfin_amd/csrc/mfx_reads.cpp
--- a/merfin_amd/csrc/mfx_reads.cpp
+++ b/merfin_amd/csrc/mfx_reads.cpp
@@ -184,6 +184,7 @@
   }
   (void)hipFree(nmeta);
   (void)hipFree(ix->d_slots);
+  mfx_index_drop_hints(ix);
   ix->d_slots = ns;
   ix->nlines = new_lines;
   ix->capacity_kmers = (uint64_t)((double)new_lines * MFX_SLOTS_LINE * 0.7);
diff --git a/merfin_amd/csrc/mfx_stream_plan.h b/merfin_amd/csrc/mfx_stream_plan.h
--- a/merfin_amd/csrc/mfx_stream_plan.h
+++ b/merfin_amd/csrc/mfx_stream_plan.h
@@ -9,6 +9,7 @@
 
 inline void seq_layout_fill(mfx_seq *s, const uint64_t *lens, uint32_t ncontigs) {
   s->ncontigs = ncontigs;
+  s->layout_hash = 0;
   s->off.resize(ncontigs);
   s->len.assign(lens, lens + ncontigs);
   s->tile_start.resize((size_t)ncontigs + 1);
```

Measured after the change: 155.8 billion. 0.985x the previous value.
